# megvii-research/Far3D

Hardware: AMD Instinct MI355X
Metric: samples/sec (7-cam frame) end-to-end @ VoV-99 640x960 (higher is better)
Workload: dtype bf16x3; 1 GPU; BASELINE configs[1]: 7 cameras 3x640x960, VoV-99, A=1544 queries (644 learned + 644 adaptive + 256 propagated), 2312 self-attn keys, 6 decoder layers, streaming memory on, ego motion on; proposals=topk, fused_rows=True, parallelism=single GPU, weights=seeded random (far3d_amd.weights.init_state_dict, seed 0)

## Files before the change

### far3d_amd/csrc/conv_ws.hip

```cpp
#include "conv_ws.hpp"
#include "far3d_hip.h"

#ifdef FAR3D_PROFILING
std::atomic<int> g_ws_ablate{0};
extern "C" int far3d_conv_ws_set_ablate(int mask) { g_ws_ablate.store(mask); return 0; }
#endif

int far3d_conv_ws_launch(const IgemmParams& P, int tile, hipStream_t st) {
  switch (tile) {
    case 400: return launch_conv3x3_ws<2, 4, 2, 2, 4, true, true>(P, st);
    case 401: return launch_conv3x3_ws<1, 8, 2, 1, 4, true, true>(P, st);
    case 402: return launch_conv3x3_ws<1, 8, 5, 1, 4, true, false>(P, st);
    case 403: return launch_conv3x3_ws<2, 4, 3, 1, 4, true, true>(P, st);
    case 404: return launch_conv3x3_ws<2, 2, 1, 2, 2, true, true>(P, st);
    case 405: return launch_conv3x3_ws<2, 4, 2, 1, 4, true, true>(P, st);
    case 406: return launch_conv3x3_ws<2, 4, 1, 2, 4, true, true>(P, st);
    case 407: return launch_conv3x3_ws<1, 4, 5, 1, 2, true, false>(P, st);
    case 408: return launch_conv3x3_ws<1, 4, 3, 1, 2, true, true>(P, st);
    case 409: return launch_conv3x3_ws<2, 4, 2, 2, 2, true, true>(P, st);
    case 410: return launch_conv3x3_ws<2, 4, 2, 2, 4, true, true, 4>(P, st);
    case 411: return launch_conv3x3_ws<2, 4, 2, 1, 4, true, true, 6>(P, st);
    case 412: return launch_conv3x3_ws<2, 4, 1, 2, 4, true, true, 8>(P, st);
    case 413: return launch_conv3x3_ws<1, 8, 2, 1, 4, true, true, 8>(P, st);
    case 414: return launch_conv3x3_ws<1, 4, 5, 1, 2, true, false, 5>(P, st);
    case 415: return launch_conv3x3_ws<2, 2, 1, 2, 2, true, true, 6>(P, st);
    case 416: return launch_conv3x3_ws<2, 4, 3, 1, 4, true, true, 4>(P, st);
    case 417: return launch_conv3x3_ws<2, 4, 2, 1, 4, true, true, 4>(P, st);
    case 418: return launch_conv3x3_ws<4, 2, 2, 2, 4, true, true, 3>(P, st);
    case 419: return launch_conv3x3_ws<4, 2, 2, 1, 4, true, true, 3>(P, st);
    case 440: return launch_conv3x3_ws<2, 4, 2, 2, 4, true, true, 3, true>(P, st);
    case 444: return launch_conv3x3_ws<2, 2, 1, 2, 2, true, true, 3, true>(P, st);
    case 445: return launch_conv3x3_ws<2, 4, 2, 1, 4, true, true, 6, true>(P, st);
    case 450: return launch_conv3x3_ws<2, 4, 2, 1, 4, true, true, 6, false, 3>(P, st);
    case 451: return launch_conv3x3_ws<2, 4, 1, 2, 4, true, true, 6, false, 3>(P, st);
    case 452: return launch_conv3x3_ws<2, 4, 1, 2, 4, true, true, 9, false, 3>(P, st);
    case 453: return launch_conv3x3_ws<1, 8, 2, 1, 4, true, true, 6, false, 3>(P, st);
    case 454: return launch_conv3x3_ws<1, 8, 2, 1, 4, true, true, 9, false, 3>(P, st);
    case 455: return launch_conv3x3_ws<1, 7, 2, 1, 4, true, true, 9, false, 3>(P, st);
    case 456: return launch_conv3x3_ws<2, 7, 1, 1, 2, true, true, 9, false, 3>(P, st);
    case 457: return launch_conv3x3_ws<2, 2, 1, 2, 2, true, true, 6, false, 3>(P, st);
    case 458: return launch_conv3x3_ws<1, 4, 3, 1, 2, true, true, 6, false, 3>(P, st);
    case 459: return launch_conv3x3_ws<2, 4, 1, 1, 4, true, true, 9, false, 3>(P, st);
    case 420: return launch_conv3x3_ws<2, 4, 2, 2, 4, false, true>(P, st);
    case 421: return launch_conv3x3_ws<1, 8, 2, 1, 4, false, true>(P, st);
    case 422: return launch_conv3x3_ws<1, 8, 5, 1, 4, false, true>(P, st);
    case 423: return launch_conv3x3_ws<2, 4, 3, 1, 4, false, true>(P, st);
    default: break;
  }
  far3d_set_error("far3d_conv2d_nhwc: unknown wave-specialised tile %d", tile);
  return FAR3D_ERR_ARG;
}

int far3d_gemm_ws_launch(const IgemmParams& P, int tile, hipStream_t st) {
  switch (tile) {
    case 460: return launch_gemm1x1_ws<4, 2, 1, 2, 4, 4, 1>(P, st);
    case 461: return launch_gemm1x1_ws<4, 2, 1, 2, 4, 4, 2>(P, st);
    case 462: return launch_gemm1x1_ws<2, 4, 2, 1, 4, 4, 2>(P, st);
    case 463: return launch_gemm1x1_ws<2, 2, 2, 2, 4, 4, 2>(P, st);
    case 464: return launch_gemm1x1_ws<4, 2, 2, 2, 4, 3, 1>(P, st);
    case 465: return launch_gemm1x1_ws<4, 2, 1, 2, 2, 4, 2>(P, st);
    case 466: return launch_gemm1x1_ws<2, 2, 1, 2, 4, 6, 3>(P, st);
    case 467: return launch_gemm1x1_ws<2, 4, 1, 1, 4, 6, 2>(P, st);
    case 468: return launch_gemm1x1_ws<2, 2, 1, 2, 2, 3, 1>(P, st);
    case 469: return launch_gemm1x1_ws<4, 2, 1, 2, 4, 2, 1>(P, st);
    case 470: return launch_gemm1x1_ws<2, 4, 2, 2, 4, 3, 1>(P, st);
    case 471: return launch_gemm1x1_ws<2, 2, 4, 2, 4, 3, 1>(P, st);
    case 473: return launch_gemm1x1_ws<4, 2, 2, 2, 2, 3, 1>(P, st);
    case 474: return launch_gemm1x1_ws<3, 2, 2, 2, 4, 3, 1>(P, st);
    case 475: return launch_gemm1x1_ws<2, 2, 2, 2, 4, 4, 1>(P, st);
    case 476: return launch_gemm1x1_ws<2, 4, 2, 2, 2, 3, 1>(P, st);
    default: break;
  }
  far3d_set_error("far3d_conv2d_nhwc: unknown wave-specialised GEMM tile %d", tile);
  return FAR3D_ERR_ARG;
}

static int far3d_conv_ws_grouped_launch(const IgemmParams& P, const WsGroup& G, int tile, hipStream_t st) {
  switch (tile) {
    case 500: return launch_conv3x3_ws_grouped<2, 4, 2, 2, 4, true, true>(P, G, st);
    case 505: return launch_conv3x3_ws_grouped<2, 4, 2, 1, 4, true, true>(P, G, st);
    case 552: return launch_conv3x3_ws_grouped<2, 4, 1, 2, 4, true, true, 9, false, 3>(P, G, st);
    case 556: return launch_conv3x3_ws_grouped<2, 7, 1, 1, 2, true, true, 9, false, 3>(P, G, st);
    case 559: return launch_conv3x3_ws_grouped<2, 4, 1, 1, 4, true, true, 9, false, 3>(P, G, st);
    default: break;
  }
  far3d_set_error("far3d_conv2d_nhwc_grouped: unknown grouped tile %d", tile);
  return FAR3D_ERR_ARG;
}

extern "C" int far3d_conv2d_nhwc_grouped(const far3d_conv_problem* probs, int n, int tile, void* stream) {
  FAR3D_CHECK_ARG(probs && n >= 1 && n <= FAR3D_WS_GROUP_MAX, "far3d_conv2d_nhwc_grouped: %d problems (1..%d)", n, FAR3D_WS_GROUP_MAX);
  FAR3D_CHECK_ARG(tile >= 500 && tile < 560, "far3d_conv2d_nhwc_grouped: tile %d is not a grouped tile (500-559)", tile);
  auto aligned = [](const void* p, long a) { return ((uintptr_t)p % a) == 0; };
  WsGroup G;
  memset(&G, 0, sizeof(G));
  G.n = n;
  const int Cin = probs[0].Cin;
  for (int i = 0; i < n; ++i) {
    const far3d_conv_problem& c = probs[i];
    FAR3D_CHECK_ARG(c.Cin == Cin, "far3d_conv2d_nhwc_grouped: problem %d has Cin %d, problem 0 has %d (one Cin per launch)", i, c.Cin, Cin);
    FAR3D_CHECK_ARG(c.x && c.w && c.y && c.N > 0 && c.H > 0 && c.W > 0 && c.Cout > 0 && Cin > 0 && Cin % 32 == 0 && c.Cout % 32 == 0 &&
                    c.act >= 0 && c.act <= 2 && c.ldx >= 2 * Cin && c.ldy >= 2 * c.Cout &&
                    aligned(c.x, 16) && aligned(c.y, 16) && c.ldx % 8 == 0 && c.ldy % 8 == 0 && c.x_img_stride % 8 == 0 && c.y_img_stride % 8 == 0 &&
                    (long)c.N * c.H * c.W < (1L << 31) - 4096 && (long)c.H * c.W * c.ldx * 2 < 0x7fffffffL,
                    "far3d_conv2d_nhwc_grouped: problem %d: needs pair-stored maps in and out, Cin and Cout multiples of 32, 16-byte aligned rows "
                    "(N=%d H=%d W=%d Cin=%d Cout=%d ldx=%d ldy=%d act=%d)", i, c.N, c.H, c.W, c.Cin, c.Cout, c.ldx, c.ldy, c.act);
    FAR3D_CHECK_ARG(!c.y2 || (c.y2_scale && c.y2_shift && aligned(c.y2, 16) && aligned(c.y2_scale, 16) && aligned(c.y2_shift, 16) &&
                              c.ldy2 >= c.Cout && c.ldy2 % 4 == 0 && c.y2_img_stride % 4 == 0),
                    "far3d_conv2d_nhwc_grouped: problem %d: the second output is fp32 with 16-byte aligned rows, scale and shift", i);
    WsProblem& q = G.p[i];
    q.x = c.x; q.w = c.w; q.bias = c.bias; q.y = c.y;
    q.y2 = c.y2; q.y2_scale = c.y2_scale; q.y2_shift = c.y2_shift;
    q.x_img_stride = c.x_img_stride; q.y_img_stride = c.y_img_stride; q.y2_img_stride = c.y2_img_stride;
    q.N = c.N; q.H = c.H; q.W = c.W; q.ldx = c.ldx; q.ldy = c.ldy; q.ldy2 = c.ldy2; q.Cout = c.Cout; q.act = c.act;
  }
  IgemmParams P;
  memset(&P, 0, sizeof(P));
  const far3d_conv_problem& c0 = probs[0];
  P.x = c0.x; P.w = c0.w; P.bias = c0.bias; P.y = c0.y;
  P.x_img_stride = c0.x_img_stride; P.y_img_stride = c0.y_img_stride;
  P.N = c0.N; P.H = c0.H; P.W = c0.W; P.Cin = Cin; P.ldx = c0.ldx; P.Ho = c0.H; P.Wo = c0.W; P.Cout = c0.Cout; P.ldy = c0.ldy;
  P.KH = 3; P.KW = 3; P.stride = 1; P.pad = 1;
  P.cin_pad = Cin; P.nsteps = 9 * Cin / 32;
  P.act = c0.act; P.y_dt = FAR3D_DT_BF16_PAIR;
  const int rc = far3d_conv_ws_grouped_launch(P, G, tile, (hipStream_t)stream);
  if (rc != FAR3D_OK) return rc;
  FAR3D_CHECK_LAUNCH("far3d_conv2d_nhwc_grouped");
  return FAR3D_OK;
}
```

### far3d_amd/csrc/conv_ws.hpp

```cpp
#pragma once
#include "igemm_kernels.hpp"
#include <type_traits>

__device__ __forceinline__ __amdgpu_buffer_rsrc_t uniform_rsrc(const void* p, long nbytes) {
  const unsigned long long a = (unsigned long long)(uintptr_t)p;
  const unsigned lo = __builtin_amdgcn_readfirstlane((unsigned)a), hi = __builtin_amdgcn_readfirstlane((unsigned)(a >> 32));
  const int nb = __builtin_amdgcn_readfirstlane((int)(nbytes < 0x7fffffffL ? nbytes : 0x7fffffffL));
  return __builtin_amdgcn_make_buffer_rsrc((void*)(uintptr_t)(((unsigned long long)hi << 32) | lo), 0, nb, 0x00020000);
}

__device__ __forceinline__ void wait_vmcnt_dyn(int n) {
#define FAR3D_WVC(k) case k: wait_vmcnt<k>(); break;
  switch (n) {
    FAR3D_WVC(0) FAR3D_WVC(1) FAR3D_WVC(2) FAR3D_WVC(3) FAR3D_WVC(4) FAR3D_WVC(5) FAR3D_WVC(6) FAR3D_WVC(7) FAR3D_WVC(8)
    FAR3D_WVC(9) FAR3D_WVC(10) FAR3D_WVC(11) FAR3D_WVC(12) FAR3D_WVC(13) FAR3D_WVC(14) FAR3D_WVC(15) FAR3D_WVC(16)
    FAR3D_WVC(17) FAR3D_WVC(18) FAR3D_WVC(19) FAR3D_WVC(20) FAR3D_WVC(21) FAR3D_WVC(22) FAR3D_WVC(23) FAR3D_WVC(24)
    FAR3D_WVC(25) FAR3D_WVC(26) FAR3D_WVC(27) FAR3D_WVC(28) FAR3D_WVC(29) FAR3D_WVC(30) FAR3D_WVC(31) FAR3D_WVC(32)
    FAR3D_WVC(33) FAR3D_WVC(34) FAR3D_WVC(35) FAR3D_WVC(36) FAR3D_WVC(37) FAR3D_WVC(38) FAR3D_WVC(39) FAR3D_WVC(40)
    FAR3D_WVC(41) FAR3D_WVC(42) FAR3D_WVC(43) FAR3D_WVC(44) FAR3D_WVC(45) FAR3D_WVC(46) FAR3D_WVC(47)
    default: wait_vmcnt<48>(); break;
  }
#undef FAR3D_WVC
}

#ifdef FAR3D_PROFILING
extern std::atomic<int> g_ws_ablate;
#define FAR3D_WS_ABLATE_ARG g_ws_ablate.load(std::memory_order_relaxed)
#else
#define FAR3D_WS_ABLATE_ARG 0
#endif

struct WsProblem {
  const void* x; const void* w; const float* bias; void* y;
  float* y2; const float* y2_scale; const float* y2_shift;
  long x_img_stride, y_img_stride, y2_img_stride;
  int N, H, W, ldx, ldy, ldy2, Cout, act;
  int tiles_x, tiles_y, n_mt, item0;
};
struct WsGroup { WsProblem p[FAR3D_WS_GROUP_MAX]; int n; };
struct WsSingle {};

template <int WGM, int WGN, int WM, int WN, int NP, bool PAIR, bool DBUF, int NSW = 3, bool FLAGS = false, int GRP = 1, class GT = WsSingle>
__global__ __launch_bounds__(64 * (WGM * WGN + NP)) void conv3x3_ws_kernel(IgemmParams P, int tiles_x, int tiles_y, int n_mt, int n_items, int ablate,
                                                                          GT GP) {
#if defined(__HIP_DEVICE_COMPILE__)
  constexpr bool GROUPED = std::is_same<GT, WsGroup>::value;
  static_assert(!GROUPED || (PAIR && !FLAGS), "grouped launches: pair storage, barrier hand-over");
  constexpr int NWC = WGM * WGN;
  static_assert(NSW >= 3, "ring depth");
  static_assert(GRP == 1 || (GRP == 3 && (NSW == 6 || NSW == 9) && !FLAGS), "one barrier per tap, or per kernel row with a ring of 2 or 3 rows");
  constexpr int NG = NSW / GRP;
  constexpr int PLD = PAIR ? 2 : 1;
  constexpr int BM = 32 * WGM * WM, TH = WGN * WN, PW = 34, PH = TH + 2, PPIX = PW * PH;
  constexpr int PG = (PPIX + 15) / 16, PATCH_B = PG * 1024;
  constexpr int GA = BM / 16, WST = BM * 64, WSTAGE = PLD * WST;
  constexpr int PBASE = NSW * WSTAGE, PBUF = PLD * PATCH_B;
  constexpr int RB = WN + 2;
  constexpr int FLAGB = PBASE + 2 * PBUF;
  static_assert(FLAGB + (FLAGS ? 128 : 0) <= 163840, "LDS budget");
  static_assert(!FLAGS || (NP <= 4 && NWC <= 8), "flag words: one b128 read per 4 counters");
  extern __shared__ __attribute__((aligned(1024))) unsigned char smem[];
  [[maybe_unused]] volatile unsigned* const flg = reinterpret_cast<volatile unsigned*>(smem + FLAGB);
  if constexpr (FLAGS) {
    if (threadIdx.x < 32) flg[threadIdx.x] = 0u;
    __syncthreads();
  }
  [[maybe_unused]] bool gave_up = false;
  constexpr int SPIN_LIMIT = 1 << 18;
  const int t = threadIdx.x, lane = t & 63, wv = __builtin_amdgcn_readfirstlane(t >> 6);
  const int nchunks = P.cin_pad / 32;
  const int spt = 9 * nchunks;
  const int my_items = (n_items - (int)blockIdx.x + (int)gridDim.x - 1) / (int)gridDim.x;
  const int total_steps = my_items * spt, total_chunks = my_items * nchunks;
  const int Ktot = 9 * P.cin_pad * PLD;
  auto locate = [&](int item, int& q, int& li, int& txs, int& tys, int& nmt) __attribute__((always_inline)) {
    q = 0; li = item; txs = tiles_x; tys = tiles_y; nmt = n_mt;
    if constexpr (GROUPED) {
      for (int i = 1; i < GP.n; ++i) q += item >= GP.p[i].item0 ? 1 : 0;
      q = __builtin_amdgcn_readfirstlane(q);
      li = item - GP.p[q].item0; txs = GP.p[q].tiles_x; tys = GP.p[q].tiles_y; nmt = GP.p[q].n_mt;
    }
  };
#ifdef FAR3D_PROFILING
  if (P.prof && t == 0) {
    unsigned hw_, xcc_;
    asm volatile("s_getreg_b32 %0, hwreg(HW_REG_HW_ID)" : "=s"(hw_));
    asm volatile("s_getreg_b32 %0, hwreg(HW_REG_XCC_ID)" : "=s"(xcc_));
    P.prof[(long)blockIdx.x * 16 + 0] = (unsigned long long)hw_ | ((unsigned long long)xcc_ << 32);
    P.prof[(long)blockIdx.x * 16 + 6] = (unsigned long long)__builtin_amdgcn_s_memrealtime();
    P.prof[(long)blockIdx.x * 16 + 1] = (unsigned long long)__builtin_amdgcn_s_memtime();
    P.prof[(long)blockIdx.x * 16 + 4] = (unsigned long long)my_items;
  }
#endif

  if (wv >= NWC) {
    const int pw = wv - NWC;
    constexpr int GPL = (PG + NP - 1) / NP, GWL = (GA + NP - 1) / NP;
    const int rg = lane >> 2, pc = lane & 3;
    const int lc = pc ^ ((rg >> 2) & 3);
    int npq = (PG - pw + NP - 1) / NP, nwq = (GA - pw + NP - 1) / NP;
    npq = npq < 0 ? 0 : npq; nwq = nwq < 0 ? 0 : nwq;
    const int np = npq * PLD, nw = nwq * PLD;
    constexpr unsigned OOB = 0x80000000u;
    unsigned wvoff[GWL];
#pragma unroll
    for (int i = 0; i < GWL; ++i) wvoff[i] = (unsigned)((((pw + NP * i) * 16 + rg) * Ktot + lc * 8) * 2);
    long img_bytes = (long)P.H * P.W * P.ldx * 2;
    unsigned pvoff[GPL];
    const bf16_t* x_base = nullptr;
    const bf16_t* w_base = nullptr;
    long w_bytes = 0;
    auto decode = [&](int k, int& n, int& y0, int& x0, int& m0, int& q) __attribute__((always_inline)) {
      const int item = (int)blockIdx.x + k * (int)gridDim.x;
      int li, txs, tys, nmt;
      locate(item, q, li, txs, tys, nmt);
      const int mt = li % nmt, pt = li / nmt;
      const int tx = pt % txs, r = pt / txs;
      const int ty = r % tys;
      n = __builtin_amdgcn_readfirstlane(r / tys); y0 = __builtin_amdgcn_readfirstlane(ty * TH);
      x0 = __builtin_amdgcn_readfirstlane(tx * 32); m0 = __builtin_amdgcn_readfirstlane(mt * BM);
    };
    auto set_w_tile = [&](int k) __attribute__((always_inline)) {
      int n, y0, x0, m0, q;
      decode(k, n, y0, x0, m0, q);
      const void* w = P.w;
      int Cout = P.Cout;
      if constexpr (GROUPED) { w = GP.p[q].w; Cout = GP.p[q].Cout; }
      w_base = reinterpret_cast<const bf16_t*>(w) + (long)m0 * Ktot;
      w_bytes = w_tile_bytes(BM, m0, Cout, Ktot);
    };
    auto set_p_tile = [&](int k) __attribute__((always_inline)) {
      int n, y0, x0, m0, q;
      decode(k, n, y0, x0, m0, q);
      const void* x = P.x;
      long xis = P.x_img_stride;
      int H = P.H, W = P.W, ldx = P.ldx;
      if constexpr (GROUPED) {
        x = GP.p[q].x; xis = GP.p[q].x_img_stride; H = GP.p[q].H; W = GP.p[q].W; ldx = GP.p[q].ldx;
        img_bytes = (long)H * W * ldx * 2;
      }
      x_base = reinterpret_cast<const bf16_t*>(x) + (long)n * xis;
#pragma unroll
      for (int i = 0; i < GPL; ++i) {
        const int idx = (pw + NP * i) * 16 + rg;
        const int py = idx / PW, px = idx - py * PW;
        const int iy = y0 - 1 + py, ix = x0 - 1 + px;
        const bool ok = idx < PPIX && iy >= 0 && iy < H && ix >= 0 && ix < W;
        pvoff[i] = ok ? (unsigned)((((long)iy * W + ix) * ldx + lc * 8) * 2) : OOB;
      }
    };
    auto issue_w = [&](int step_in_tile, int stage) __attribute__((always_inline)) {
      const int c = step_in_tile / 9, tap = step_in_tile - 9 * c;
      const int kb = __builtin_amdgcn_readfirstlane((tap * P.cin_pad + c * 32) * PLD * 2);
      const __amdgpu_buffer_rsrc_t rs_w = uniform_rsrc(w_base, w_bytes);
      const int sbase = __builtin_amdgcn_readfirstlane(stage * WSTAGE);
#pragma unroll
      for (int i = 0; i < GWL; ++i) {
        if (i < nwq) {
#pragma unroll
          for (int pl = 0; pl < PLD; ++pl)
            __builtin_amdgcn_raw_ptr_buffer_load_lds(rs_w, (lds_void_t*)(smem + sbase + pl * WST + (pw + NP * i) * 1024), 16, wvoff[i],
                                                     kb + pl * 64, 0, 0);
        }
      }
    };
    auto issue_p = [&](int chunk_in_tile, int buf) __attribute__((always_inline)) {
      const __amdgpu_buffer_rsrc_t rs_x = uniform_rsrc(x_base, img_bytes);
      const int pbase = __builtin_amdgcn_readfirstlane(PBASE + buf * PBUF), coff = __builtin_amdgcn_readfirstlane(chunk_in_tile * (64 * PLD));
#pragma unroll
      for (int i = 0; i < GPL; ++i) {
        if (i < npq) {
#pragma unroll
          for (int pl = 0; pl < PLD; ++pl)
            __builtin_amdgcn_raw_ptr_buffer_load_lds(rs_x, (lds_void_t*)(smem + pbase + pl * PATCH_B + (pw + NP * i) * 1024), 16, pvoff[i],
                                                     coff + pl * 64, 0, 0);
        }
      }
    };
    int sw_step = 0, sw_tile = 0, sw_stage = 0;
    int gp_chunk = 0, gp_tile = 0, gp_buf = 0;
    int w_left = total_steps, p_left = total_chunks;
    set_w_tile(0); set_p_tile(0);
    auto next_w = [&]() __attribute__((always_inline)) {
      if (!(ablate & 1)) issue_w(sw_step, sw_stage);
      --w_left;
      sw_stage = sw_stage == NSW - 1 ? 0 : sw_stage + 1;
      if (++sw_step == spt) { sw_step = 0; ++sw_tile; if (w_left > 0) set_w_tile(sw_tile); }
    };
    auto next_p = [&]() __attribute__((always_inline)) {
      if (!(ablate & 1)) issue_p(gp_chunk, gp_buf);
      --p_left;
      gp_buf ^= 1;
      if (++gp_chunk == nchunks) { gp_chunk = 0; ++gp_tile; if (p_left > 0) set_p_tile(gp_tile); }
    };
    next_p();
#pragma unroll
    for (int i = 0; i < (NG - 1) * GRP; ++i)
      if (w_left > 0) next_w();
    const int total_groups = total_steps / GRP, gpc = 9 / GRP;
    int gic = 0;
    unsigned phist = 0;
    for (int g = 0; g < total_groups; ++g) {
      int ahead = total_groups - 1 - g;
      ahead = ahead > NG - 2 ? NG - 2 : ahead;
      const int cnt = ahead * GRP * nw + __builtin_popcount(phist & ((1u << (NG - 1)) - 1u)) * np;
      const int S = g * GRP;
      if (ablate & 1) wait_vmcnt<0>(); else wait_vmcnt_dyn(cnt);
      if constexpr (FLAGS) {
        if (lane == 0) flg[pw] = (unsigned)(S + 1);
        if (S > 0 && !(ablate & 8)) {
          for (int spins = 0; !gave_up; ++spins) {
            const u32x4_t c0 = *reinterpret_cast<volatile u32x4_t*>(smem + FLAGB + 64);
            u32x4_t c1 = c0;
            if constexpr (NWC > 4) c1 = *reinterpret_cast<volatile u32x4_t*>(smem + FLAGB + 80);
            unsigned m = c0.x;
            if constexpr (NWC > 1) m = min(m, c0.y);
            if constexpr (NWC > 2) m = min(m, c0.z);
            if constexpr (NWC > 3) m = min(m, c0.w);
            if constexpr (NWC > 4) m = min(m, c1.x);
            if constexpr (NWC > 5) m = min(m, c1.y);
            if constexpr (NWC > 6) m = min(m, c1.z);
            if constexpr (NWC > 7) m = min(m, c1.w);
            if (__builtin_amdgcn_readfirstlane(m) >= (unsigned)S) break;
            if (spins > SPIN_LIMIT) gave_up = true;
            __builtin_amdgcn_s_sleep(2);
          }
        }
      } else {
#ifdef FAR3D_PROFILING
        if (!(ablate & 8))
#endif
        __builtin_amdgcn_s_barrier();
      }
      asm volatile("" ::: "memory");
#pragma unroll
      for (int i = 0; i < GRP; ++i)
        if (w_left > 0) next_w();
      phist <<= 1;
      if (gic == 0 && p_left > 0) { next_p(); phist |= 1u; }
      gic = gic == gpc - 1 ? 0 : gic + 1;
    }
    return;
  }

  const int wm = wv / WGN, wn = wv % WGN, l31 = lane & 31, hi = lane >> 5;
  int aaddr[WM], baddr[RB][3];
#pragma unroll
  for (int i = 0; i < WM; ++i) {
    const int r = (wm * WM + i) * 32 + l31;
    aaddr[i] = r * 64 + ((hi ^ ((r >> 2) & 3)) << 4);
  }
#pragma unroll
  for (int r = 0; r < RB; ++r)
#pragma unroll
    for (int kx = 0; kx < 3; ++kx) {
      const int idx = (wn * WN + r) * PW + l31 + kx;
      baddr[r][kx] = PBASE + idx * 64 + ((hi ^ ((idx >> 2) & 3)) << 4);
    }
  f32x16_t acc[WM][WN];
  u32x4_t fa[2][PLD][WM], fb[2][PLD][WN];

  auto load_a = [&](int set, int soff, int kk) __attribute__((always_inline)) {
#ifdef FAR3D_PROFILING
    if (ablate & 4) return;
#endif
    const int x32 = kk * 32;
#pragma unroll
    for (int pl = 0; pl < PLD; ++pl)
#pragma unroll
      for (int i = 0; i < WM; ++i) fa[set][pl][i] = *reinterpret_cast<const u32x4_t*>(smem + pl * WST + ((aaddr[i] ^ x32) + soff));
  };
  auto load_b = [&](int set, int tap, int kk) __attribute__((always_inline)) {
#ifdef FAR3D_PROFILING
    if (ablate & 4) return;
#endif
    const int ky = tap / 3, kx = tap - 3 * ky, x32 = kk * 32;
#pragma unroll
    for (int pl = 0; pl < PLD; ++pl)
#pragma unroll
      for (int j = 0; j < WN; ++j) fb[set][pl][j] = *reinterpret_cast<const u32x4_t*>(smem + pl * PATCH_B + (baddr[j + ky][kx] ^ x32));
  };
  auto load_set = [&](int set, int soff, int tap, int kk) __attribute__((always_inline)) { load_a(set, soff, kk); load_b(set, tap, kk); };
  auto mma_term = [&](int set, int term) __attribute__((always_inline)) {
    const int pa = (PAIR && term == 0) ? 1 : 0, pb = (PAIR && term == 1) ? 1 : 0;
#pragma unroll
    for (int i = 0; i < WM; ++i)
#pragma unroll
      for (int j = 0; j < WN; ++j) mma<bf16_t>(acc[i][j], fa[set][pa][i], fb[set][pb][j]);
  };
  auto mma_set = [&](int set) __attribute__((always_inline)) {
    if constexpr (PAIR) { mma_term(set, 0); mma_term(set, 1); }
    mma_term(set, 2);
  };

  int G = 0;
  int soff = 0;
  [[maybe_unused]] int Sg = 0;
  [[maybe_unused]] u32x4_t pfl = {0u, 0u, 0u, 0u};
#ifdef FAR3D_PROFILING
  unsigned long long pf_ta = 0, pf_tb = 0, pf_wait = 0, pf_body = 0, pf_epi = 0;
  const bool pf_on = P.prof != nullptr && wv == 0;
#endif
  for (int k = 0; k < my_items; ++k) {
    const int item = (int)blockIdx.x + k * (int)gridDim.x;
    int prob, li, txs, tys, nmt;
    locate(item, prob, li, txs, tys, nmt);
    const int mt = li % nmt, pt = li / nmt;
    const int tx = pt % txs, rr = pt / txs;
    const int ty = rr % tys, n = rr / tys;
    const int x0 = tx * 32, y0 = ty * TH, m0 = mt * BM;
#pragma unroll
    for (int i = 0; i < WM; ++i)
#pragma unroll
      for (int j = 0; j < WN; ++j)
#pragma unroll
        for (int r = 0; r < 16; ++r) acc[i][j][r] = 0.f;

    for (int c = 0; c < nchunks; ++c, ++G) {
#pragma unroll
      for (int tap = 0; tap < 9; ++tap) {
        const int stage = soff;
        if (tap % GRP == 0) {
        __builtin_amdgcn_s_waitcnt(0xc07f);
#ifdef FAR3D_PROFILING
        if (pf_on) {
          const unsigned long long now = __builtin_amdgcn_s_memtime();
          if (pf_tb) { pf_wait += pf_tb - pf_ta; pf_body += now - pf_tb; }
          pf_ta = now;
        }
#endif
        if constexpr (FLAGS) {
          if (lane == 0) flg[16 + wv] = (unsigned)Sg;
          if (!(ablate & 8)) {
            for (int spins = 0; !gave_up; ++spins) {
              unsigned m = pfl.x;
              if constexpr (NP > 1) m = min(m, pfl.y);
              if constexpr (NP > 2) m = min(m, pfl.z);
              if constexpr (NP > 3) m = min(m, pfl.w);
              if (__builtin_amdgcn_readfirstlane(m) >= (unsigned)(Sg + 1)) break;
              if (spins > SPIN_LIMIT) gave_up = true;
              __builtin_amdgcn_s_sleep(1);
              pfl = *reinterpret_cast<volatile u32x4_t*>(smem + FLAGB);
            }
          }
          ++Sg;
        } else {
#ifdef FAR3D_PROFILING
          if (!(ablate & 8))
#endif
          __builtin_amdgcn_s_barrier();
        }
        asm volatile("" ::: "memory");
        __builtin_amdgcn_sched_barrier(0);
#ifdef FAR3D_PROFILING
        if (pf_on) pf_tb = __builtin_amdgcn_s_memtime();
        if (tap == 0 && c == 0 && k == 0 && P.prof && t == 0) P.prof[(long)blockIdx.x * 16 + 2] = (unsigned long long)__builtin_amdgcn_s_memtime();
#endif
        }
        if (ablate & 2) { soff = soff == (NSW - 1) * WSTAGE ? 0 : soff + WSTAGE; continue; }
        if constexpr (DBUF) {
          load_set(0, stage, tap, 0);
          __builtin_amdgcn_sched_barrier(0);
          if (tap > 0 || c > 0) mma_set(1);
          __builtin_amdgcn_sched_barrier(0);
          load_a(1, stage, 1);
          if constexpr (FLAGS) pfl = *reinterpret_cast<volatile u32x4_t*>(smem + FLAGB);
          __builtin_amdgcn_sched_barrier(0);
          if constexpr (PAIR) {
            mma_term(0, 0);
            __builtin_amdgcn_sched_barrier(0);
            load_b(1, tap, 1);
            __builtin_amdgcn_sched_barrier(0);
            mma_term(0, 1);
            mma_term(0, 2);
          } else {
            load_b(1, tap, 1);
            __builtin_amdgcn_sched_barrier(0);
            mma_term(0, 2);
          }
          __builtin_amdgcn_sched_barrier(0);
          soff = soff == (NSW - 1) * WSTAGE ? 0 : soff + WSTAGE;
        } else {
          load_set(0, stage, tap, 0);
          __builtin_amdgcn_sched_barrier(0);
          mma_set(0);
          __builtin_amdgcn_sched_barrier(0);
          load_set(0, stage, tap, 1);
          if constexpr (FLAGS) pfl = *reinterpret_cast<volatile u32x4_t*>(smem + FLAGB);
          __builtin_amdgcn_sched_barrier(0);
          mma_set(0);
          __builtin_amdgcn_sched_barrier(0);
          soff = soff == (NSW - 1) * WSTAGE ? 0 : soff + WSTAGE;
        }
      }
      const int d = (G & 1) ? -PBUF : PBUF;
#pragma unroll
      for (int r = 0; r < RB; ++r)
#pragma unroll
        for (int kx = 0; kx < 3; ++kx) baddr[r][kx] += d;
    }
    if constexpr (DBUF) mma_set(1);
    __builtin_amdgcn_sched_barrier(0);
#ifdef FAR3D_PROFILING
    unsigned long long pf_e0 = 0;
    if (pf_on) {
      pf_e0 = __builtin_amdgcn_s_memtime();
      if (pf_tb) { pf_wait += pf_tb - pf_ta; pf_body += pf_e0 - pf_tb; pf_tb = 0; }
    }
#endif

    {
      const int px = x0 + l31;
      void* y = P.y;
      const float* bias = P.bias;
      long yis = P.y_img_stride;
      int Ho = P.Ho, Wo = P.Wo, ldy = P.ldy, Cout = P.Cout, act = P.act;
      [[maybe_unused]] float* y2 = nullptr;
      [[maybe_unused]] const float *y2s = nullptr, *y2h = nullptr;
      [[maybe_unused]] long y2is = 0;
      [[maybe_unused]] int ldy2 = 0;
      if constexpr (GROUPED) {
        const WsProblem& pq = GP.p[prob];
        y = pq.y; bias = pq.bias; yis = pq.y_img_stride; Ho = pq.H; Wo = pq.W; ldy = pq.ldy; Cout = pq.Cout; act = pq.act;
        y2 = pq.y2; y2s = pq.y2_scale; y2h = pq.y2_shift; y2is = pq.y2_img_stride; ldy2 = pq.ldy2;
      }
      unsigned char* yb = reinterpret_cast<unsigned char*>(y);
#pragma unroll
      for (int j = 0; j < WN; ++j) {
        const int py = y0 + wn * WN + j;
        const bool ok = py < Ho && px < Wo;
        const long pix_b = ((long)n * yis + ((long)py * Wo + px) * ldy) * 2;
#pragma unroll
        for (int i = 0; i < WM; ++i) {
          const int cb = m0 + (wm * WM + i) * 32;
          if (cb >= Cout) continue;
#pragma unroll
          for (int qp = 0; qp < 2; ++qp) {
            uint2 h[2], l[2];
#pragma unroll
            for (int u = 0; u < 2; ++u) {
              const int q = 2 * qp + u;
              float4 b4 = make_float4(0.f, 0.f, 0.f, 0.f);
              if (bias) b4 = *reinterpret_cast<const float4*>(bias + cb + 8 * q + 4 * hi);
              float v[4];
#pragma unroll
              for (int e = 0; e < 4; ++e) v[e] = acc[i][j][4 * q + e];
              v[0] += b4.x; v[1] += b4.y; v[2] += b4.z; v[3] += b4.w;
              if (act == ACT_RELU) {
#pragma unroll
                for (int e = 0; e < 4; ++e) v[e] = fmaxf(v[e], 0.f);
              } else if (act == ACT_SWISH) {
                if constexpr (PAIR) {
#pragma unroll
                  for (int e = 0; e < 4; ++e) v[e] = v[e] * (1.f / (1.f + expf(-v[e])));
                } else {
#pragma unroll
                  for (int e = 0; e < 4; ++e) v[e] = v[e] * __frcp_rn(1.f + __expf(-v[e]));
                }
              }
              if constexpr (GROUPED) {
                if (y2 && ok) {
                  const int m = cb + 8 * q + 4 * hi;
                  const long so = (long)n * Cout + m;
                  float w4[4];
#pragma unroll
                  for (int e = 0; e < 4; ++e) w4[e] = y2s[so + e] * v[e] + y2h[so + e];
                  *reinterpret_cast<float4*>(y2 + n * y2is + ((long)py * Wo + px) * ldy2 + m) = make_float4(w4[0], w4[1], w4[2], w4[3]);
                }
              }
              if constexpr (PAIR) split4f(v[0], v[1], v[2], v[3], h[u], l[u]);
              else { h[u] = make_uint2(pack_bf16x2(v[0], v[1]), pack_bf16x2(v[2], v[3])); l[u] = make_uint2(0u, 0u); }
            }
            u32x4_t oh, ol;
            {
              const auto sx = __builtin_amdgcn_permlane32_swap(h[0].x, h[1].x, false, false);
              const auto sy = __builtin_amdgcn_permlane32_swap(h[0].y, h[1].y, false, false);
              oh = u32x4_t{sx[0], sy[0], sx[1], sy[1]};
            }
            const int qoff = (2 * qp + hi) * 16;
            if constexpr (PAIR) {
              const auto sx = __builtin_amdgcn_permlane32_swap(l[0].x, l[1].x, false, false);
              const auto sy = __builtin_amdgcn_permlane32_swap(l[0].y, l[1].y, false, false);
              ol = u32x4_t{sx[0], sy[0], sx[1], sy[1]};
              if (ok) {
                unsigned char* d = yb + pix_b + (long)(cb >> 5) * 128 + qoff;
                *reinterpret_cast<u32x4_t*>(d) = oh;
                *reinterpret_cast<u32x4_t*>(d + 64) = ol;
              }
            } else {
              if (ok) *reinterpret_cast<u32x4_t*>(yb + pix_b + (long)cb * 2 + qoff) = oh;
            }
          }
        }
      }
    }
#ifdef FAR3D_PROFILING
    if (pf_on) pf_epi += __builtin_amdgcn_s_memtime() - pf_e0;
#endif
  }
#ifdef FAR3D_PROFILING
  if (P.prof && t == 0) {
    P.prof[(long)blockIdx.x * 16 + 3] = (unsigned long long)__builtin_amdgcn_s_memtime();
    P.prof[(long)blockIdx.x * 16 + 7] = (unsigned long long)__builtin_amdgcn_s_memrealtime();
    P.prof[(long)blockIdx.x * 16 + 5] = (unsigned long long)total_steps;
    P.prof[(long)blockIdx.x * 16 + 8] = pf_wait; P.prof[(long)blockIdx.x * 16 + 9] = pf_body; P.prof[(long)blockIdx.x * 16 + 10] = pf_epi;
  }
#endif
#endif
}

template <int WGM, int WGN, int WM, int WN, int NP, int NSW, int GRP, bool SUMS>
__global__ __launch_bounds__(64 * (WGM * WGN + NP)) void gemm1x1_ws_kernel(IgemmParams P, int npt, int nct, int ablate) {
#if defined(__HIP_DEVICE_COMPILE__)
  constexpr int NWC = WGM * WGN;
  constexpr int BM = 32 * WGM * WM, BP = 32 * WGN * WN;
  constexpr int GA = BM / 16, GB = BP / 16, SLOTS = GA + GB;
  static_assert(SLOTS % NP == 0, "every producer issues the same number of pieces per step (counted vmcnt)");
  constexpr int SPW = SLOTS / NP;
  constexpr int SUB = (BM + BP) * 64, STAGE = 2 * SUB;
  static_assert(NSW % GRP == 0 && NSW / GRP >= 2, "ring = at least two hand-over groups");
  constexpr int NG = NSW / GRP;
  extern __shared__ __attribute__((aligned(1024))) unsigned char smem[];
  const int t = threadIdx.x, lane = t & 63, wv = __builtin_amdgcn_readfirstlane(t >> 6);
  constexpr int SUMB = NSW * STAGE;
  static_assert(SUMB + 4 * BM * 8 <= 163840, "LDS budget");
  [[maybe_unused]] long long* const lsum = reinterpret_cast<long long*>(smem + SUMB);
  constexpr bool do_sums = SUMS;
  if (do_sums) {
    for (int i = threadIdx.x; i < 4 * BM; i += 64 * (NWC + NP)) lsum[i] = 0;
    __syncthreads();
  }
  const int HoWo = P.Ho * P.Wo;
  const long Npix = (long)P.N * HoWo;
  const int nsteps = P.cin_pad / 32;
  const int Ktot = P.cin_pad * 2;
  const int xcd = (int)blockIdx.x & 7, slot0 = (int)blockIdx.x >> 3, dslot = (int)gridDim.x >> 3;
  const int vslots = ((npt - xcd + 7) >> 3) * nct;
  const int my_items = vslots > slot0 ? (vslots - slot0 + dslot - 1) / dslot : 0;
  const int total_steps = my_items * nsteps;
  const int total_groups = (total_steps + GRP - 1) / GRP;
  auto decode = [&](int k, int& p0, int& m0) __attribute__((always_inline)) {
    const int slot = slot0 + k * dslot;
    const int ct = slot % nct, pt = (slot / nct) * 8 + xcd;
    p0 = __builtin_amdgcn_readfirstlane(pt * BP); m0 = __builtin_amdgcn_readfirstlane(ct * BM);
  };

  if (wv >= NWC) {
    const int pw = wv - NWC;
    const int rg = lane >> 2, pc = lane & 3;
    const int lc = pc ^ ((rg >> 2) & 3);
    constexpr unsigned OOB = 0x80000000u;
    const long x_bytes = ((long)(P.N - 1) * P.x_img_stride + (long)HoWo * P.ldx) * 2;
    unsigned voff[SPW];
    int sdst[SPW];
    bool isw[SPW];
#pragma unroll
    for (int i = 0; i < SPW; ++i) {
      const int q = pw + NP * i;
      isw[i] = q < GA;
      const int g = isw[i] ? q : q - GA;
      sdst[i] = (isw[i] ? 0 : BM * 64) + g * 1024;
      voff[i] = isw[i] ? (unsigned)(((g * 16 + rg) * Ktot + lc * 8) * 2) : 0u;
    }
    const bf16_t* w_base = nullptr;
    long w_bytes = 0;
    int cur_tile = 0, cur_step = 0, cur_stage = 0, left = total_steps;
    auto set_tile = [&](int k) __attribute__((always_inline)) {
      int p0, m0;
      decode(k, p0, m0);
      w_base = reinterpret_cast<const bf16_t*>(P.w) + (long)m0 * Ktot;
      w_bytes = w_tile_bytes(BM, m0, P.Cout, Ktot);
#pragma unroll
      for (int i = 0; i < SPW; ++i) {
        if (!isw[i]) {
          const int g = pw + NP * i - GA;
          const long p = (long)p0 + g * 16 + rg;
          if (p < Npix) {
            int n, rem;
            pix_split(p, HoWo, n, rem);
            voff[i] = (unsigned)(((long)n * P.x_img_stride + (long)rem * P.ldx + lc * 8) * 2);
          } else {
            voff[i] = OOB;
          }
        }
      }
    };
    auto next = [&]() __attribute__((always_inline)) {
      if (!(ablate & 1)) {
        const __amdgpu_buffer_rsrc_t rs_w = uniform_rsrc(w_base, w_bytes);
        const __amdgpu_buffer_rsrc_t rs_x = uniform_rsrc(P.x, x_bytes);
        const int sbase = __builtin_amdgcn_readfirstlane(cur_stage * STAGE);
        const int kb = __builtin_amdgcn_readfirstlane(cur_step * 128);
#pragma unroll
        for (int i = 0; i < SPW; ++i) {
#pragma unroll
          for (int pl = 0; pl < 2; ++pl) {
            if (isw[i])
              __builtin_amdgcn_raw_ptr_buffer_load_lds(rs_w, (lds_void_t*)(smem + sbase + pl * SUB + sdst[i]), 16, voff[i], kb + pl * 64, 0, 0);
            else
              __builtin_amdgcn_raw_ptr_buffer_load_lds(rs_x, (lds_void_t*)(smem + sbase + pl * SUB + sdst[i]), 16, voff[i], kb + pl * 64, 0, 0);
          }
        }
      }
      --left;
      cur_stage = cur_stage == NSW - 1 ? 0 : cur_stage + 1;
      if (++cur_step == nsteps) { cur_step = 0; ++cur_tile; if (left > 0) set_tile(cur_tile); }
    };
    if (my_items > 0) set_tile(0);
#pragma unroll
    for (int i = 0; i < (NG - 1) * GRP; ++i)
      if (left > 0) next();
    for (int g = 0; g < total_groups; ++g) {
      int later = total_steps - (g + 1) * GRP;
      later = later < 0 ? 0 : (later > (NG - 2) * GRP ? (NG - 2) * GRP : later);
      if (ablate & 1) wait_vmcnt<0>(); else wait_vmcnt_dyn(later * SPW * 2);
      __builtin_amdgcn_s_barrier();
      asm volatile("" ::: "memory");
#pragma unroll
      for (int i = 0; i < GRP; ++i)
        if (left > 0) next();
    }
    if (do_sums) __builtin_amdgcn_s_barrier();
    return;
  }

  const int wm = wv / WGN, wn = wv % WGN, l31 = lane & 31, hi = lane >> 5;
  int aaddr[WM], baddr[WN];
#pragma unroll
  for (int i = 0; i < WM; ++i) {
    const int r = (wm * WM + i) * 32 + l31;
    aaddr[i] = r * 64 + ((hi ^ ((r >> 2) & 3)) << 4);
  }
#pragma unroll
  for (int j = 0; j < WN; ++j) {
    const int r = (wn * WN + j) * 32 + l31;
    baddr[j] = BM * 64 + r * 64 + ((hi ^ ((r >> 2) & 3)) << 4);
  }
  f32x16_t acc[WM][WN];
  u32x4_t fa[2][2][WM], fb[2][2][WN];
  auto load_a = [&](int set, int soff, int kk) __attribute__((always_inline)) {
    const int x32 = kk * 32;
#pragma unroll
    for (int pl = 0; pl < 2; ++pl)
#pragma unroll
      for (int i = 0; i < WM; ++i) fa[set][pl][i] = *reinterpret_cast<const u32x4_t*>(smem + pl * SUB + ((aaddr[i] ^ x32) + soff));
  };
  auto load_b = [&](int set, int soff, int kk) __attribute__((always_inline)) {
    const int x32 = kk * 32;
#pragma unroll
    for (int pl = 0; pl < 2; ++pl)
#pragma unroll
      for (int j = 0; j < WN; ++j) fb[set][pl][j] = *reinterpret_cast<const u32x4_t*>(smem + pl * SUB + ((baddr[j] ^ x32) + soff));
  };
  auto mma_term = [&](int set, int term) __attribute__((always_inline)) {
    const int pa = term == 0 ? 1 : 0, pb = term == 1 ? 1 : 0;
#pragma unroll
    for (int i = 0; i < WM; ++i)
#pragma unroll
      for (int j = 0; j < WN; ++j) mma<bf16_t>(acc[i][j], fa[set][pa][i], fb[set][pb][j]);
  };
  int soff = 0, gs = 0;
  [[maybe_unused]] int flush_tile = 0, gcount = 0;
  auto flush = [&](int T) __attribute__((always_inline)) {
    int fp0, fm0;
    decode(T, fp0, fm0);
    const int fcam0 = (int)((long)fp0 / P.sums_hw);
    long long* src = lsum + (T & 1) * 2 * BM;
    for (int i = wv * 64 + lane; i < 2 * BM; i += 64 * NWC) {
      const int sl = i / BM, chn = i - sl * BM, cam = fcam0 + sl;
      const long long v = src[i];
      if (v != 0) {
        src[i] = 0;
        if (cam < P.N && fm0 + chn < P.Cout)
          atomicAdd(reinterpret_cast<unsigned long long*>(P.chan_sums + (long)cam * P.Cout + fm0 + chn), (unsigned long long)v);
      }
    }
  };
  for (int k = 0; k < my_items; ++k) {
    int p0, m0;
    decode(k, p0, m0);
#pragma unroll
    for (int i = 0; i < WM; ++i)
#pragma unroll
      for (int j = 0; j < WN; ++j)
#pragma unroll
        for (int r = 0; r < 16; ++r) acc[i][j][r] = 0.f;
    for (int s = 0; s < nsteps; ++s) {
      const int stage = soff;
      if (gs == 0) {
        __builtin_amdgcn_s_waitcnt(0xc07f);
        __builtin_amdgcn_s_barrier();
        asm volatile("" ::: "memory");
        __builtin_amdgcn_sched_barrier(0);
        if constexpr (do_sums) {
          while (flush_tile < k && ((flush_tile + 1) * nsteps - 1) / GRP < gcount) { flush(flush_tile); ++flush_tile; }
          ++gcount;
        }
      }
      gs = gs == GRP - 1 ? 0 : gs + 1;
      if (ablate & 2) { soff = soff == (NSW - 1) * STAGE ? 0 : soff + STAGE; continue; }
      load_a(0, stage, 0); load_b(0, stage, 0);
      __builtin_amdgcn_sched_barrier(0);
      if (s > 0) { mma_term(1, 0); mma_term(1, 1); mma_term(1, 2); }
      __builtin_amdgcn_sched_barrier(0);
      load_a(1, stage, 1);
      __builtin_amdgcn_sched_barrier(0);
      mma_term(0, 0);
      __builtin_amdgcn_sched_barrier(0);
      load_b(1, stage, 1);
      __builtin_amdgcn_sched_barrier(0);
      mma_term(0, 1);
      mma_term(0, 2);
      __builtin_amdgcn_sched_barrier(0);
      soff = soff == (NSW - 1) * STAGE ? 0 : soff + STAGE;
    }
    if (!(ablate & 2)) { mma_term(1, 0); mma_term(1, 1); mma_term(1, 2); }
    __builtin_amdgcn_sched_barrier(0);

    {
      unsigned char* yb = reinterpret_cast<unsigned char*>(P.y);
      const int cam0 = do_sums ? (int)((long)p0 / P.sums_hw) : 0;
      const long bnd = (long)(cam0 + 1) * P.sums_hw;
      const bool two = do_sums && (long)p0 + BP > bnd;
      long pix_b[WN];
      bool okj[WN], secj[WN];
#pragma unroll
      for (int j = 0; j < WN; ++j) {
        const long p = (long)p0 + (wn * WN + j) * 32 + l31;
        okj[j] = p < Npix;
        secj[j] = p >= bnd;
        pix_b[j] = 0;
        if (okj[j]) {
          int n, rem;
          pix_split(p, HoWo, n, rem);
          pix_b[j] = ((long)n * P.y_img_stride + (long)rem * P.ldy) * 2;
        }
      }
      auto stored = [&](int i, int j, int q, int cb, uint2& h, uint2& l) __attribute__((always_inline)) {
        float4 b4 = make_float4(0.f, 0.f, 0.f, 0.f);
        if (P.bias) b4 = *reinterpret_cast<const float4*>(P.bias + cb + 8 * q + 4 * hi);
        float v[4];
#pragma unroll
        for (int e = 0; e < 4; ++e) v[e] = acc[i][j][4 * q + e];
        v[0] += b4.x; v[1] += b4.y; v[2] += b4.z; v[3] += b4.w;
        if (P.act == ACT_RELU) {
#pragma unroll
          for (int e = 0; e < 4; ++e) v[e] = fmaxf(v[e], 0.f);
        } else if (P.act == ACT_SWISH) {
#pragma unroll
          for (int e = 0; e < 4; ++e) v[e] = v[e] * (1.f / (1.f + expf(-v[e])));
        }
        split4f(v[0], v[1], v[2], v[3], h, l);
      };
      auto quantise = [&](const uint2& h, const uint2& l, int q, int (&qs)[16], float& mx) __attribute__((always_inline)) {
        const unsigned w4[4] = {h.x, h.y, l.x, l.y};
#pragma unroll
        for (int e = 0; e < 2; ++e) {
          const float h0 = __uint_as_float(w4[e] << 16), h1 = __uint_as_float(w4[e] & 0xffff0000u);
          const float l0 = __uint_as_float(w4[2 + e] << 16), l1 = __uint_as_float(w4[2 + e] & 0xffff0000u);
          mx = fmaxf(mx, fmaxf(fabsf(h0), fabsf(h1)));
          qs[4 * q + 2 * e] += __float2int_rn(h0 * (float)(1 << FAR3D_SUMS_FRAC_BITS)) + __float2int_rn(l0 * (float)(1 << FAR3D_SUMS_FRAC_BITS));
          qs[4 * q + 2 * e + 1] += __float2int_rn(h1 * (float)(1 << FAR3D_SUMS_FRAC_BITS)) + __float2int_rn(l1 * (float)(1 << FAR3D_SUMS_FRAC_BITS));
        }
      };
      auto half_sum = [&](int x) __attribute__((always_inline)) -> int {
        x += __builtin_amdgcn_update_dpp(0, x, 0x128, 0xf, 0xf, true);
        x += __builtin_amdgcn_update_dpp(0, x, 0x124, 0xf, 0xf, true);
        x += __builtin_amdgcn_update_dpp(0, x, 0x122, 0xf, 0xf, true);
        x += __builtin_amdgcn_update_dpp(0, x, 0x121, 0xf, 0xf, true);
        typedef unsigned u2_t __attribute__((ext_vector_type(2)));
        const u2_t r = __builtin_amdgcn_permlane16_swap((unsigned)x, (unsigned)x, false, false);
        const unsigned rx = r.x, ry = r.y;
        return (int)(rx + ry);
      };
      auto reduce_add = [&](const int (&qs)[16], float mx, int sl, int cb) __attribute__((always_inline)) {
        const bool wide = WN > 2 || __any(mx >= (float)(1 << (24 - FAR3D_SUMS_FRAC_BITS)));
        long long* dst = lsum + ((k & 1) * 2 + sl) * BM + (cb - m0) + 4 * hi;
#pragma unroll
        for (int r = 0; r < 16; ++r) {
          long long tot;
          if (!wide) {
            tot = (long long)half_sum(qs[r]);
          } else {
            const int lo16 = qs[r] & 0xffff, hi16 = qs[r] >> 16;
            tot = (long long)half_sum(hi16) * 65536ll + (long long)half_sum(lo16);
          }
          if (l31 == 0 && tot != 0) atomicAdd(reinterpret_cast<unsigned long long*>(dst + 8 * (r >> 2) + (r & 3)), (unsigned long long)tot);
        }
      };
      auto channel_block = [&](auto ic) __attribute__((always_inline)) {
        constexpr int i = decltype(ic)::value;
        const int cb = m0 + (wm * WM + i) * 32;
        if (cb >= P.Cout) return;
        int qs[16];
        float mx = 0.f;
#pragma unroll
        for (int r = 0; r < 16; ++r) qs[r] = 0;
#pragma unroll
        for (int j = 0; j < WN; ++j) {
#pragma unroll
          for (int qp = 0; qp < 2; ++qp) {
            uint2 h[2], l[2];
#pragma unroll
            for (int u = 0; u < 2; ++u) {
              stored(i, j, 2 * qp + u, cb, h[u], l[u]);
              if (do_sums && okj[j] && !secj[j]) quantise(h[u], l[u], 2 * qp + u, qs, mx);
            }
            u32x4_t oh, ol;
            {
              const auto sx = __builtin_amdgcn_permlane32_swap(h[0].x, h[1].x, false, false);
              const auto sy = __builtin_amdgcn_permlane32_swap(h[0].y, h[1].y, false, false);
              oh = u32x4_t{sx[0], sy[0], sx[1], sy[1]};
            }
            {
              const auto sx = __builtin_amdgcn_permlane32_swap(l[0].x, l[1].x, false, false);
              const auto sy = __builtin_amdgcn_permlane32_swap(l[0].y, l[1].y, false, false);
              ol = u32x4_t{sx[0], sy[0], sx[1], sy[1]};
            }
            if (okj[j]) {
              unsigned char* d = yb + pix_b[j] + (long)(cb >> 5) * 128 + (2 * qp + hi) * 16;
              *reinterpret_cast<u32x4_t*>(d) = oh;
              *reinterpret_cast<u32x4_t*>(d + 64) = ol;
            }
          }
        }
        if constexpr (do_sums) {
          auto exact_add = [&](int sl) __attribute__((always_inline)) {
            long long* dst = lsum + ((k & 1) * 2 + sl) * BM + (cb - m0) + 4 * hi;
#pragma unroll
            for (int q = 0; q < 4; ++q) {
              long long x[4] = {0, 0, 0, 0};
#pragma unroll
              for (int j = 0; j < WN; ++j) {
                uint2 h, l;
                stored(i, j, q, cb, h, l);
                if (okj[j] && secj[j] == (sl == 1)) {
                  const unsigned w4[4] = {h.x, h.y, l.x, l.y};
#pragma unroll
                  for (int e = 0; e < 2; ++e) {
                    const float h0 = __uint_as_float(w4[e] << 16), h1 = __uint_as_float(w4[e] & 0xffff0000u);
                    const float l0 = __uint_as_float(w4[2 + e] << 16), l1 = __uint_as_float(w4[2 + e] & 0xffff0000u);
                    x[2 * e] += __double2ll_rn((double)h0 * (double)(1 << FAR3D_SUMS_FRAC_BITS)) + __double2ll_rn((double)l0 * (double)(1 << FAR3D_SUMS_FRAC_BITS));
                    x[2 * e + 1] += __double2ll_rn((double)h1 * (double)(1 << FAR3D_SUMS_FRAC_BITS)) + __double2ll_rn((double)l1 * (double)(1 << FAR3D_SUMS_FRAC_BITS));
                  }
                }
              }
#pragma unroll
              for (int e = 0; e < 4; ++e) {
                const long long v = x[e];
                const long long tot = (long long)half_sum((int)(v & 0xffff)) + ((long long)half_sum((int)((v >> 16) & 0xffff)) << 16) +
                                      ((long long)half_sum((int)((v >> 32) & 0xffff)) << 32) + ((long long)half_sum((int)(v >> 48)) << 48);
                if (l31 == 0 && tot != 0) atomicAdd(reinterpret_cast<unsigned long long*>(dst + 8 * q + e), (unsigned long long)tot);
              }
            }
          };
          const bool huge = __any(mx >= 2048.f);
          if (huge) exact_add(0); else reduce_add(qs, mx, 0, cb);
          if (two) {
            float mx1 = 0.f;
#pragma unroll
            for (int r = 0; r < 16; ++r) qs[r] = 0;
#pragma unroll
            for (int j = 0; j < WN; ++j)
#pragma unroll
              for (int q = 0; q < 4; ++q) {
                uint2 h, l;
                stored(i, j, q, cb, h, l);
                if (okj[j] && secj[j]) quantise(h, l, q, qs, mx1);
              }
            if (__any(mx1 >= 2048.f)) exact_add(1); else reduce_add(qs, mx1, 1, cb);
          }
        }
      };
      static_assert(WM <= 4, "channel blocks per consumer");
      channel_block(std::integral_constant<int, 0>{});
      if constexpr (WM > 1) channel_block(std::integral_constant<int, 1>{});
      if constexpr (WM > 2) channel_block(std::integral_constant<int, 2>{});
      if constexpr (WM > 3) channel_block(std::integral_constant<int, 3>{});
    }
  }
  if constexpr (do_sums) {
    __builtin_amdgcn_s_waitcnt(0xc07f);
    __builtin_amdgcn_s_barrier();
    asm volatile("" ::: "memory");
    while (flush_tile < my_items) { flush(flush_tile); ++flush_tile; }
  }
#endif
}

template <int WGM, int WGN, int WM, int WN, int NP, int NSW, int GRP>
static int launch_gemm1x1_ws(const IgemmParams& P, hipStream_t st) {
  constexpr int BM = 32 * WGM * WM, BP = 32 * WGN * WN;
  constexpr size_t lds = (size_t)NSW * 2 * (BM + BP) * 64 + 4 * BM * 8;
  static_assert(lds <= 163840, "LDS budget");
  const long Npix = (long)P.N * P.Ho * P.Wo;
  const int npt = (int)((Npix + BP - 1) / BP), nct = (P.Cout + BM - 1) / BM;
  static std::atomic<unsigned long long> lds_ok_s{0};
  static std::atomic<int> n_cu{0};
  int cus = n_cu.load(std::memory_order_relaxed);
  if (cus == 0) {
    int dev = 0;
    if (hipGetDevice(&dev) != hipSuccess) dev = 0;
    if (hipDeviceGetAttribute(&cus, hipDeviceAttributeMultiprocessorCount, dev) != hipSuccess || cus <= 0) cus = 256;
    n_cu.store(cus, std::memory_order_relaxed);
  }
  constexpr int wg_per_cu = lds <= 81920 && 64 * (WGM * WGN + NP) <= 1024 ? 2 : 1;
  const long items = (long)((npt + 7) / 8 * 8) * nct;
  long grid = (long)cus * wg_per_cu;
  grid = (grid + 7) / 8 * 8;
  if (items < grid) grid = items;
  static std::atomic<unsigned long long> lds_ok{0};
  if constexpr (lds > 65536)
    if (const int rc = far3d_allow_lds(P.chan_sums ? reinterpret_cast<const void*>(&gemm1x1_ws_kernel<WGM, WGN, WM, WN, NP, NSW, GRP, true>)
                                                   : reinterpret_cast<const void*>(&gemm1x1_ws_kernel<WGM, WGN, WM, WN, NP, NSW, GRP, false>),
                                       (int)lds, P.chan_sums ? lds_ok_s : lds_ok, "far3d_conv2d_nhwc")) return rc;
  if (P.chan_sums) {
    if (P.sums_hw < BP || P.cin_pad / 32 < 2 * GRP) {
      far3d_set_error("far3d_conv2d_nhwc: channel sums on this wave-specialised GEMM tile need Ho*Wo (%d) >= %d pixels and Cin >= %d", P.sums_hw, BP, 64 * GRP);
      return FAR3D_ERR_ARG;
    }
    hipLaunchKernelGGL((gemm1x1_ws_kernel<WGM, WGN, WM, WN, NP, NSW, GRP, true>), dim3((unsigned)grid), dim3(64 * (WGM * WGN + NP)), lds, st, P, npt, nct, FAR3D_WS_ABLATE_ARG);
  } else {
    hipLaunchKernelGGL((gemm1x1_ws_kernel<WGM, WGN, WM, WN, NP, NSW, GRP, false>), dim3((unsigned)grid), dim3(64 * (WGM * WGN + NP)), lds, st, P, npt, nct, FAR3D_WS_ABLATE_ARG);
  }
  return 0;
}

template <int WGM, int WGN, int WM, int WN, int NP, bool PAIR, bool DBUF, int NSW = 3, bool FLAGS = false, int GRP = 1>
static int launch_conv3x3_ws(const IgemmParams& P, hipStream_t st) {
  constexpr int BM = 32 * WGM * WM, TH = WGN * WN, PLD = PAIR ? 2 : 1;
  constexpr int PG = (34 * (TH + 2) + 15) / 16;
  constexpr size_t lds = (size_t)NSW * PLD * BM * 64 + (size_t)2 * PLD * PG * 1024 + (FLAGS ? 128 : 0);
  static_assert(lds <= 163840, "LDS budget");
  const int tiles_x = (P.Wo + 31) / 32, tiles_y = (P.Ho + TH - 1) / TH, n_mt = (P.Cout + BM - 1) / BM;
  const int n_items = P.N * tiles_x * tiles_y * n_mt;
  static std::atomic<int> n_cu{0};
  int cus = n_cu.load(std::memory_order_relaxed);
  if (cus == 0) {
    int dev = 0;
    if (hipGetDevice(&dev) != hipSuccess) dev = 0;
    if (hipDeviceGetAttribute(&cus, hipDeviceAttributeMultiprocessorCount, dev) != hipSuccess || cus <= 0) cus = 256;
    n_cu.store(cus, std::memory_order_relaxed);
  }
  constexpr int wg_per_cu = lds <= 81920 && 64 * (WGM * WGN + NP) <= 1024 ? 2 : 1;
  const int grid = n_items < cus * wg_per_cu ? n_items : cus * wg_per_cu;
  static std::atomic<unsigned long long> lds_ok{0};
  if constexpr (lds > 65536)
    if (const int rc = far3d_allow_lds(reinterpret_cast<const void*>(&conv3x3_ws_kernel<WGM, WGN, WM, WN, NP, PAIR, DBUF, NSW, FLAGS, GRP>), (int)lds, lds_ok, "far3d_conv2d_nhwc")) return rc;
  hipLaunchKernelGGL((conv3x3_ws_kernel<WGM, WGN, WM, WN, NP, PAIR, DBUF, NSW, FLAGS, GRP>), dim3((unsigned)grid), dim3(64 * (WGM * WGN + NP)), lds, st, P, tiles_x, tiles_y, n_mt,
                     n_items, FAR3D_WS_ABLATE_ARG, WsSingle{});
  return 0;
}

template <int WGM, int WGN, int WM, int WN, int NP, bool PAIR, bool DBUF, int NSW = 3, bool FLAGS = false, int GRP = 1>
static int launch_conv3x3_ws_grouped(const IgemmParams& P, const WsGroup& G0, hipStream_t st) {
  constexpr int BM = 32 * WGM * WM, TH = WGN * WN, PLD = PAIR ? 2 : 1;
  constexpr int PG = (34 * (TH + 2) + 15) / 16;
  constexpr size_t lds = (size_t)NSW * PLD * BM * 64 + (size_t)2 * PLD * PG * 1024 + (FLAGS ? 128 : 0);
  static_assert(lds <= 163840, "LDS budget");
  WsGroup G = G0;
  long items[FAR3D_WS_GROUP_MAX];
  for (int i = 0; i < G.n; ++i) {
    WsProblem& q = G.p[i];
    q.tiles_x = (q.W + 31) / 32; q.tiles_y = (q.H + TH - 1) / TH; q.n_mt = (q.Cout + BM - 1) / BM;
    items[i] = (long)q.N * q.tiles_x * q.tiles_y * q.n_mt;
  }
  for (int i = 1; i < G.n; ++i)
    for (int j = i; j > 0 && items[j] > items[j - 1]; --j) {
      const WsProblem t = G.p[j]; G.p[j] = G.p[j - 1]; G.p[j - 1] = t;
      const long u = items[j]; items[j] = items[j - 1]; items[j - 1] = u;
    }
  long n_items = 0;
  for (int i = 0; i < G.n; ++i) { G.p[i].item0 = (int)n_items; n_items += items[i]; }
  if (n_items >= (1L << 31) - 4096) { far3d_set_error("far3d_conv2d_nhwc_grouped: %ld items", n_items); return FAR3D_ERR_ARG; }
  static std::atomic<int> n_cu{0};
  int cus = n_cu.load(std::memory_order_relaxed);
  if (cus == 0) {
    int dev = 0;
    if (hipGetDevice(&dev) != hipSuccess) dev = 0;
    if (hipDeviceGetAttribute(&cus, hipDeviceAttributeMultiprocessorCount, dev) != hipSuccess || cus <= 0) cus = 256;
    n_cu.store(cus, std::memory_order_relaxed);
  }
  constexpr int wg_per_cu = lds <= 81920 && 64 * (WGM * WGN + NP) <= 1024 ? 2 : 1;
  const int grid = n_items < cus * wg_per_cu ? (int)n_items : cus * wg_per_cu;
  static std::atomic<unsigned long long> lds_ok{0};
  if constexpr (lds > 65536)
    if (const int rc = far3d_allow_lds(reinterpret_cast<const void*>(&conv3x3_ws_kernel<WGM, WGN, WM, WN, NP, PAIR, DBUF, NSW, FLAGS, GRP, WsGroup>), (int)lds, lds_ok,
                                       "far3d_conv2d_nhwc_grouped")) return rc;
  hipLaunchKernelGGL((conv3x3_ws_kernel<WGM, WGN, WM, WN, NP, PAIR, DBUF, NSW, FLAGS, GRP, WsGroup>), dim3((unsigned)grid), dim3(64 * (WGM * WGN + NP)), lds, st, P,
                     G.p[0].tiles_x, G.p[0].tiles_y, G.p[0].n_mt, (int)n_items, FAR3D_WS_ABLATE_ARG, G);
  return 0;
}
```

### far3d_amd/lib.py

```python
import ctypes
import os

os.environ.setdefault("GPU_MAX_HW_QUEUES", "8")

import torch

_HERE = os.path.dirname(os.path.abspath(__file__))
LIB_PATH = os.path.join(_HERE, "libfar3d_hip.so")

c_int, c_float, c_void_p, c_char_p = ctypes.c_int, ctypes.c_float, ctypes.c_void_p, ctypes.c_char_p
c_long = ctypes.c_long
_p = c_void_p

SIGNATURES = {
    "far3d_last_error": (c_char_p, []),
    "far3d_abi_version": (c_int, []),
    "far3d_device_count": (c_int, []),
    "far3d_device_arch": (c_int, [c_int, c_char_p, c_int]),
    "far3d_msda_forward": (c_int, [_p, c_int, _p, _p, _p, _p, _p] + [c_int] * 7 + [_p]),
    "far3d_aggregate_forward": (c_int, [_p, c_int, _p, _p, _p, _p, _p, _p, _p, _p, c_int] + [c_int] * 7 +
                                [_p, _p, _p, c_float, c_float, c_int, c_int, c_int, _p, _p, c_int, _p, _p]),
    "far3d_conv2d_nhwc": (c_int, [_p, c_int, _p, c_int, _p, _p, c_int] + [c_int] * 5 + [c_long] + [c_int] * 4 +
                          [c_long] + [c_int] * 5 + [_p, c_int, c_int, c_long, c_int, c_int] +
                          [_p, c_int, c_int, c_long, _p, _p, _p, c_int, _p]),
    "far3d_conv2d_nhwc_grouped": (c_int, [_p, c_int, c_int, _p]),
    "far3d_attention_forward": (c_int, [_p, _p, _p, c_int, _p, c_int] + [c_int] * 8 + [c_float, _p, c_int, c_int, _p]),
    "far3d_attention_f32_variant": (c_int, [c_int]),
    "far3d_layernorm": (c_int, [_p, _p, _p, _p, c_int, c_int, c_int, c_int, c_float, c_int, _p, c_int, _p, c_int, c_int, _p, c_int, c_int, _p]),
    "far3d_layernorm_rows": (c_int, [_p, _p, _p, _p, c_int, c_int, c_int, c_int, c_float, c_int, _p, c_int, _p, c_int, c_int, _p, c_int, c_int, _p, _p]),
    "far3d_rowchain_attn_out": (c_int, [_p, c_int, _p, c_int, _p, c_int, _p, _p, _p, _p, _p, _p, c_int, _p, c_int, _p, c_int,
                                        _p, c_int, c_float, _p]),
    "far3d_rowchain_ffn": (c_int, [_p, c_int, _p, c_int, _p, c_int] + [_p] * 12 + [_p, c_int, _p, c_int, _p, c_int, c_int, c_float, _p]),
    "far3d_rowchain_qkv": (c_int, [_p, c_int, _p, c_int, _p, _p, _p, c_int, c_int, _p]),
    "far3d_rowchain_branches": (c_int, [_p, c_int] + [_p] * 10 + [c_int] + [_p] * 6 + [c_int, _p, c_int, _p, c_int, c_int, c_float, _p]),
    "far3d_ese_nhwc": (c_int, [_p, c_int, _p, _p, _p, _p, _p, c_int, c_int, c_int, c_int, c_long, c_int, c_long,
                               c_int, c_long, _p, _p]),
    "far3d_ese_fused_nhwc": (c_int, [_p, c_int, _p, _p, _p, _p, _p, _p, c_int, c_int, c_int, c_int, c_int, c_long, c_int, c_long, c_int, c_long,
                                     c_int, c_int, c_int, c_long, _p, _p]),
    "far3d_cam_embed_chain": (c_int, [_p] * 10 + [c_int, c_int, c_int, c_int, c_float, c_int, _p]),
    "far3d_groupnorm_nhwc": (c_int, [_p, c_int, _p, _p, _p, _p, c_int, c_int, c_int, c_int, c_float, c_int, _p]),
    "far3d_maxpool3x3s2_nhwc": (c_int, [_p, c_int, _p] + [c_int] * 7 + [c_long, _p]),
    "far3d_stem_im2col": (c_int, [_p, _p, c_int, c_int, c_int, c_int, _p]),
    "far3d_stem_conv": (c_int, [_p, _p, _p, _p, c_int, c_int, c_int, c_int, c_long, c_int, _p]),
    "far3d_proposal_select": (c_int, [_p, _p, c_int, c_int, c_int, c_int, _p, _p, _p, _p, _p, _p, c_int, c_float, c_int, _p]),
    "far3d_proposal_gather": (c_int, [_p, c_int, c_int, c_int, _p, _p, _p, _p, c_int, _p, _p, c_int, c_int, c_int, c_int,
                                      c_float, c_float, c_int, _p, _p, c_int, c_int, _p, c_float, _p, _p, _p, _p, c_int, _p, _p, _p]),
    "far3d_proposal_gather_md": (c_int, [_p, c_int, c_int, c_int, _p, _p, _p, _p, c_int, _p, _p, c_int, c_int, c_int, c_int,
                                         c_float, c_float, c_int, _p, _p, c_int, c_int, _p, c_float, _p, _p, _p, _p, c_int,
                                         c_int, c_int, _p, _p, _p]),
    "far3d_proposal_extra_rows": (c_int, [_p, c_int, c_int, c_int, c_int, _p, _p, _p, c_float, c_float, c_int, _p, c_int,
                                          _p, _p, _p, _p, c_int, c_int, _p, _p, _p]),
    "far3d_compact_rows": (c_int, [_p, _p, c_int, c_int, c_int, _p, c_int, _p, _p, _p]),
    "far3d_row_affine_ln": (c_int, [_p, _p, _p, _p, _p] + [c_int] * 6 + [c_float, c_int, _p]),
    "far3d_posemb3d": (c_int, [_p, _p, _p, c_int, _p]),
    "far3d_memory_prepare": (c_int, [_p] * 9 + [c_float, c_int, _p, c_int, c_int, c_int] + [_p] * 9),
    "far3d_head_finalize": (c_int, [_p] * 5 + [c_int] * 4 + [_p, _p, c_int, c_int, _p]),
    "far3d_memory_post_update": (c_int, [_p] * 10 + [c_int] * 4 + [_p] * 6),
    "far3d_add_cast": (c_int, [_p, _p, _p, c_int, _p, c_int, c_int, c_int, c_long, c_long, _p]),
    "far3d_agg_order": (c_int, [_p, _p, _p, c_int, c_int, _p, c_float, c_float, _p, c_int, c_int, c_int, _p, _p, c_int, c_int, c_int, _p, _p, _p]),
    "far3d_agg_tables": (c_int, [_p, _p, c_int, c_int, c_int, _p]),
    "far3d_topk": (c_int, [_p, c_int, c_int, _p, _p, _p]),
    "far3d_decode_topk": (c_int, [_p, _p, c_int, c_int, c_int, c_int, _p, _p, _p, _p, _p, _p, c_long, _p]),
    "far3d_decode_topk_mem": (c_int, [_p, _p, c_int, c_int, c_int, c_int, _p, _p, _p, _p, _p, _p, c_long, _p, c_int, c_int, _p, _p]),
    "far3d_camera_prep": (c_int, [_p, _p, _p, _p, _p, c_int, _p]),
    "far3d_nan_to_num": (c_int, [_p, _p, c_long, _p]),
    "far3d_image_resample_h": (c_int, [_p, c_long, c_int, c_int, _p, _p, _p, c_int, c_int, c_int, c_int, c_int, _p]),
    "far3d_image_resample_v": (c_int, [_p, c_int, c_int, c_int, _p, _p, c_int, c_int, c_int, c_int, c_int, _p, c_int, c_int, c_int,
                                       _p, _p, c_int, _p]),
}

_lib = None


class Far3dHipError(RuntimeError):
    pass


def load():
    global _lib
    if _lib is not None:
        return _lib
    if not os.path.exists(LIB_PATH):
        raise Far3dHipError(
            "libfar3d_hip.so not found at %s -- run `python -c 'import __graft_entry__ as g; g.build()'` "
            "(or `python far3d_amd/build.py`). There is no CPU fallback for the Far3D hot path." % LIB_PATH)
    lib = ctypes.CDLL(LIB_PATH)
    for name, (res, args) in SIGNATURES.items():
        fn = getattr(lib, name)
        fn.restype = res
        fn.argtypes = args
    _lib = lib
    return lib


def check(status, what):
    if status != 0:
        msg = load().far3d_last_error()
        raise Far3dHipError("%s failed (code %d): %s" % (what, status, msg.decode() if msg else "?"))


def require_device():
    lib = load()
    if lib.far3d_device_count() <= 0:
        raise Far3dHipError("far3d_amd needs a HIP device (MI355X / gfx950); none is visible and there is "
                            "no CPU fallback. The CPU restatement lives in oracle/ and is test-only.")
    return lib
```

### include/far3d_hip.h

```cpp
#ifndef FAR3D_HIP_H
#define FAR3D_HIP_H
#include <stdint.h>

#ifdef __cplusplus
extern "C" {
#endif

#define FAR3D_DT_F32 0
#define FAR3D_DT_BF16 1
#define FAR3D_DT_F32_BF16X3 2
#define FAR3D_DT_BF16_PAIR 3
#define FAR3D_SUMS_MAX_PARTS 32
#define FAR3D_SUMS_FRAC_BITS 18
#define FAR3D_SUMS_SCRATCH_FLOATS(N, C) ((long)(N) * (C) * (2 * FAR3D_SUMS_MAX_PARTS + 1))

#define FAR3D_OK 0
#define FAR3D_ERR_ARG (-1)
#define FAR3D_ERR_LAUNCH (-2)
#define FAR3D_ERR_UNSUPPORTED (-3)

const char* far3d_last_error(void);
int far3d_abi_version(void);
int far3d_device_count(void);
int far3d_device_arch(int dev, char* buf, int buflen);

int far3d_msda_forward(const void* value, int value_dtype, const int64_t* spatial_shapes,
                       const int64_t* level_start_index, const float* sampling_loc,
                       const float* attn_weight, float* out, int bs, int S, int H, int Dh, int L, int Q,
                       int P, void* stream);

int far3d_aggregate_forward(const void* feat, int feat_dtype, const float* ref, const float* offsets,
                            const float* lidar2img, const float* U, const float* Vc, const float* cam_tables,
                            const int32_t* perm, void* out, int out_dt, int A,
                            int N, int S, int C, int G, int P, int L, const int32_t* level_hw,
                            const int32_t* level_start, const float* pc_range, float pad_h, float pad_w,
                            int ldU, int ldOffs, int variant, float* split_partials, int32_t* split_tickets, int split_extra,
                            const float* qbase, void* stream);
#define FAR3D_AGG_LISTS_FLOATS(A) ((long)(((A) + 7) / 8 * 8) * (2L * 1024 * 9 + 8))

int far3d_agg_tables(const float* Vc, float* tables, int layers, int N, int J, void* stream);

int far3d_conv2d_nhwc(const void* x, int x_dt, const void* w, int w_dt, const float* bias, void* y, int y_dt,
                      int N, int H, int W, int Cin, int ldx, long x_img_stride, int Ho, int Wo, int Cout, int ldy,
                      long y_img_stride, int KH, int KW, int stride, int pad, int act, const void* res, int res_dt,
                      int ldr, long res_img_stride, int Hr, int Wr, void* y2, int y2_dt, int ldy2,
                      long y2_img_stride, const float* y2_scale, const float* y2_shift, long long* chan_sums, int tile,
                      void* stream);

typedef struct {
  const void* x;
  const void* w;
  const float* bias;
  void* y;
  float* y2;
  const float* y2_scale;
  const float* y2_shift;
  long x_img_stride, y_img_stride, y2_img_stride;
  int N, H, W, Cin, Cout, ldx, ldy, ldy2;
  int act;
} far3d_conv_problem;
#define FAR3D_WS_GROUP_MAX 16

int far3d_conv2d_nhwc_grouped(const far3d_conv_problem* probs, int n, int tile, void* stream);

int far3d_attention_forward(const void* q, const void* k, const void* v, int dtype, void* out, int out_dt, int Aq, int Nk,
                            int heads, int head_dim, int ldq, int ldk, int ldv, int ldo, float scale,
                            const int32_t* hole_count, int hole_start, int hole_end, void* stream);

int far3d_attention_f32_variant(int variant);

int far3d_layernorm(const float* x, const float* gamma, const float* beta, float* y, int rows, int C, int ldx,
                    int ldy, float eps, int act, const float* add, int lda, void* y2, int ldy2, int y2_dt, void* yb, int ldyb,
                    int yb_dt, void* stream);
int far3d_layernorm_rows(const float* x, const float* gamma, const float* beta, float* y, int rows, int C, int ldx,
                         int ldy, float eps, int act, const float* add, int lda, void* y2, int ldy2, int y2_dt, void* yb, int ldyb,
                         int yb_dt, const int32_t* out_rows, void* stream);

int far3d_rowchain_attn_out(const void* att, int ld_att, const float* x, int ldx, const float* qpos, int ldq,
                            const void* w_out, const float* b_out, const float* g0, const float* be0,
                            const void* w_wl, const float* b_wl, int n_wl, float* x1, int ldx1, float* ul, int ldu,
                            const int32_t* ul_rows, int M, float eps, void* stream);

int far3d_rowchain_ffn(const void* agg, int ld_agg, const float* x1, int ldx1, const float* qpos, int ldq,
                       const void* w_o, const float* b_o, const float* g1, const float* be1,
                       const void* w_1, const float* b_1, const void* w_2, const float* b_2,
                       const float* g2, const float* be2, const void* w_qkv, const float* b_qkv,
                       float* out, int ldo, void* qkv, int ldqkv, void* xop, int ldxop, int M, float eps, void* stream);

int far3d_rowchain_qkv(const float* x, int ldx, const float* qpos, int ldq, const void* w_qkv, const float* b_qkv,
                       void* qkv, int ldqkv, int M, void* stream);

int far3d_rowchain_branches(const void* h, int ldh, const void* w_c0, const float* b_c0, const float* g_c0, const float* be_c0,
                            const void* w_c1, const float* b_c1, const float* g_c1, const float* be_c1,
                            const void* w_c2, const float* b_c2, int n_cls, const void* w_r0, const float* b_r0,
                            const void* w_r1, const float* b_r1, const void* w_r2, const float* b_r2, int n_reg,
                            float* cls, int ld_cls, float* reg, int ld_reg, int M, float eps, void* stream);

int far3d_ese_nhwc(const void* x, int dt, const float* fcw, const float* fcb, const void* identity, void* y,
                   float* scratch, int N, int HW, int C, int ldx, long x_img_stride, int ldi, long i_img_stride,
                   int ldy, long y_img_stride, long long* chan_sums, void* stream);

int far3d_ese_fused_nhwc(const void* x, int dt, const float* fcw, const float* fcb, const void* identity, void* y, void* pooled,
                         float* gate, int N, int H, int W, int C, int ldx, long x_img_stride, int ldi,
                         long i_img_stride, int ldy, long y_img_stride, int Hp, int Wp, int ldp, long p_img_stride,
                         long long* chan_sums, void* stream);

int far3d_groupnorm_nhwc(const void* x, int dt, const float* gamma, const float* beta, void* y, float* scratch, int N,
                         int HW, int C, int groups, float eps, int relu, void* stream);

int far3d_maxpool3x3s2_nhwc(const void* x, int dt, void* y, int N, int H, int W, int C, int Ho, int Wo, int ldy,
                            long y_img_stride, void* stream);

int far3d_stem_im2col(const float* img, void* out, int out_dt, int N, int H, int W, void* stream);

int far3d_stem_conv(const float* img, const void* w, const float* bias, void* y, int N, int H, int W, int ldy, long y_img_stride,
                    int act, void* stream);

int far3d_proposal_select(const float* const* cls, const float* const* reg, int ncls, int nreg, int N, int L,
                          const int32_t* level_hw, const int32_t* strides, float* scratch_sw, float* weights, int* sel_idx,
                          int* sel_cnt, int cap, float thr, int mode, void* stream);

int far3d_proposal_gather(const float* const* reg, int nreg, int N, int L, const int32_t* level_hw, const int32_t* strides,
                          const int* sel_idx, const int* sel_cnt, int cap, const float* weights,
                          const float* depth_logit, int hd, int wd, int nd, int depth_stride, float depth_min,
                          float depth_max, int depth_bins, const float* img2lidar, const void* feat, int feat_dt, int C,
                          const float* pc_range, float score_thr, float* ref2d, float* ctx, float* box2d, float* score,
                          int rows_total, int32_t* m_out, int32_t* overflow_out, void* stream);

int far3d_proposal_gather_md(const float* const* reg, int nreg, int N, int L, const int32_t* level_hw, const int32_t* strides,
                             const int* sel_idx, const int* sel_cnt, int cap, const float* weights,
                             const float* depth_logit, int hd, int wd, int nd, int depth_stride, float depth_min,
                             float depth_max, int depth_bins, const float* img2lidar, const void* feat, int feat_dt, int C,
                             const float* pc_range, float score_thr, float* ref2d, float* ctx, float* box2d, float* score,
                             int primary_rows, int topk, int range_min_bin, int32_t* md_flags, int32_t* md_info, void* stream);

int far3d_proposal_extra_rows(const int* sel_cnt, int N, int sel_cap, int primary_rows, int topk, const int32_t* md_flags,
                              const int32_t* md_info, const float* img2lidar, float depth_min, float depth_max, int depth_bins,
                              const float* pc_range, int C, float* ref2d, float* ctx, float* box2d, float* score, int rows_total,
                              int fill_hole, int32_t* m_out, int32_t* overflow_out, void* stream);

int far3d_compact_rows(const float* src, const int32_t* counts, int nblocks, int rows_per_block, int D, float* dst, int dst_rows,
                       int32_t* m_out, int32_t* overflow_out, void* stream);

int far3d_row_affine_ln(const float* x, const float* gamma, const float* beta, const float* add, float* y, int rows, int C,
                        int ldx, int ldg, int lda, int ldy, float eps, int do_ln, void* stream);


int far3d_posemb3d(const float* pos, const float* dim_t128, float* out, int R, void* stream);

int far3d_memory_prepare(const float* emb, const float* ref, const double* ts, const float* pose, const float* velo,
                         const float* ego_pose_inv, const double* timestamp, const float* pseudo_ref, const float* dim_t256,
                         float prev_exists, int fresh, const float* pc_range, int L, int E, int P, float* m_emb, float* m_ref,
                         double* m_ts, float* m_pose, float* m_velo, float* temp_ref, float* nerf, float* tpos, void* stream);

int far3d_head_finalize(const float* reg, const float* ref, float* cls_all, float* box, float* score, int layers, int A,
                        int code_size, int num_classes, const float* pc_range, const int32_t* hole_count, int hole_start, int hole_end,
                        void* stream);

int far3d_memory_post_update(const float* m_emb, const float* m_ref, const double* m_ts, const float* m_pose, const float* m_velo,
                             const int64_t* topk_idx, const float* dec_last, const float* box_last, const float* ego_pose,
                             const double* timestamp, int L, int E, int K, int code_size, float* emb, float* ref, double* ts,
                             float* pose, float* velo, void* stream);

int far3d_add_cast(const float* a, const float* b, void* out_sum, int sum_dt, void* out_a, int a_dt, int rows, int C, long ld_sum,
                   long ld_a, void* stream);

int far3d_agg_order(const float* ref, const float* lidar2img, int32_t* perm, int A, int N, const float* pc_range, float pad_h,
                    float pad_w, const int32_t* hole_count, int hole_start, int hole_end, int row_base,
                    const float* Vc, float* tables, int layers, int J, int split_extra, int32_t* inv, float* qbase, void* stream);

int far3d_topk(const float* vals, int n, int K, int64_t* idx_out, float* val_out, void* stream);

#define FAR3D_DECODE_WS_BYTES(n, K) ((((long)(n) + 40959) / 40960) * (long)(K) * 8)
int far3d_decode_topk(const float* cls_last, const float* box_last, int A, int num_classes, int code_size, int K,
                      const float* post_center_range, float* boxes, float* scores, int64_t* labels, unsigned char* keep,
                      void* workspace, long workspace_bytes, void* stream);
int far3d_decode_topk_mem(const float* cls_last, const float* box_last, int A, int num_classes, int code_size, int K,
                          const float* post_center_range, float* boxes, float* scores, int64_t* labels, unsigned char* keep,
                          void* workspace, long workspace_bytes, const float* mem_scores, int mem_n, int mem_K,
                          int64_t* mem_idx_out, void* stream);

int far3d_camera_prep(const float* lidar2img, const float* intrinsics, const float* extrinsics, float* img2lidar, float* c14,
                      int N, void* stream);

int far3d_nan_to_num(float* x, void* bf16_copy, long n, void* stream);

int far3d_cam_embed_chain(const float* l2i, const float* w0t, const float* b0, const float* w2t, const float* b2,
                          const float* ln_g, const float* ln_b, const float* w3t, const float* b3, float* out, int N, int L,
                          int J, int Hd, float eps, int ld_l2i, void* stream);

int far3d_image_resample_h(const unsigned char* src, long src_pitch, int in_h, int in_w, unsigned char* dst, const int32_t* bounds,
                           const int32_t* coeffs, int ksize, int row0, int rows, int x0, int outw, void* stream);
int far3d_image_resample_v(const unsigned char* tmp, int row0, int rows, int outw, const int32_t* bounds, const int32_t* coeffs,
                           int ksize, int y0, int outh, int flip, int mode, void* out, int out_dt, int pad_h, int pad_w,
                           const float* mean, const float* stdinv, int to_rgb, void* stream);

#ifdef __cplusplus
}
#endif
#endif
```

Before: 72.26 samples/s.

## Defer conv epilogue across items and deal partial Cout tiles to balance work

```diff
diff --git a/far3d_amd/csrc/conv_ws.hip b/far3d_amd/csrc/conv_ws.hip
--- a/far3d_amd/csrc/conv_ws.hip
+++ b/far3d_amd/csrc/conv_ws.hip
@@ -12,18 +12,18 @@
     case 401: return launch_conv3x3_ws<1, 8, 2, 1, 4, true, true>(P, st);
     case 402: return launch_conv3x3_ws<1, 8, 5, 1, 4, true, false>(P, st);
     case 403: return launch_conv3x3_ws<2, 4, 3, 1, 4, true, true>(P, st);
-    case 404: return launch_conv3x3_ws<2, 2, 1, 2, 2, true, true>(P, st);
-    case 405: return launch_conv3x3_ws<2, 4, 2, 1, 4, true, true>(P, st);
-    case 406: return launch_conv3x3_ws<2, 4, 1, 2, 4, true, true>(P, st);
+    case 404: return launch_conv3x3_ws<2, 2, 1, 2, 2, true, true, 3, false, 1, true>(P, st);
+    case 405: return launch_conv3x3_ws<2, 4, 2, 1, 4, true, true, 3, false, 1, true>(P, st);
+    case 406: return launch_conv3x3_ws<2, 4, 1, 2, 4, true, true, 3, false, 1, true>(P, st);
     case 407: return launch_conv3x3_ws<1, 4, 5, 1, 2, true, false>(P, st);
     case 408: return launch_conv3x3_ws<1, 4, 3, 1, 2, true, true>(P, st);
     case 409: return launch_conv3x3_ws<2, 4, 2, 2, 2, true, true>(P, st);
     case 410: return launch_conv3x3_ws<2, 4, 2, 2, 4, true, true, 4>(P, st);
     case 411: return launch_conv3x3_ws<2, 4, 2, 1, 4, true, true, 6>(P, st);
-    case 412: return launch_conv3x3_ws<2, 4, 1, 2, 4, true, true, 8>(P, st);
+    case 412: return launch_conv3x3_ws<2, 4, 1, 2, 4, true, true, 8, false, 1, true>(P, st);
     case 413: return launch_conv3x3_ws<1, 8, 2, 1, 4, true, true, 8>(P, st);
     case 414: return launch_conv3x3_ws<1, 4, 5, 1, 2, true, false, 5>(P, st);
-    case 415: return launch_conv3x3_ws<2, 2, 1, 2, 2, true, true, 6>(P, st);
+    case 415: return launch_conv3x3_ws<2, 2, 1, 2, 2, true, true, 6, false, 1, true>(P, st);
     case 416: return launch_conv3x3_ws<2, 4, 3, 1, 4, true, true, 4>(P, st);
     case 417: return launch_conv3x3_ws<2, 4, 2, 1, 4, true, true, 4>(P, st);
     case 418: return launch_conv3x3_ws<4, 2, 2, 2, 4, true, true, 3>(P, st);
@@ -31,24 +31,29 @@
     case 440: return launch_conv3x3_ws<2, 4, 2, 2, 4, true, true, 3, true>(P, st);
     case 444: return launch_conv3x3_ws<2, 2, 1, 2, 2, true, true, 3, true>(P, st);
     case 445: return launch_conv3x3_ws<2, 4, 2, 1, 4, true, true, 6, true>(P, st);
-    case 450: return launch_conv3x3_ws<2, 4, 2, 1, 4, true, true, 6, false, 3>(P, st);
-    case 451: return launch_conv3x3_ws<2, 4, 1, 2, 4, true, true, 6, false, 3>(P, st);
-    case 452: return launch_conv3x3_ws<2, 4, 1, 2, 4, true, true, 9, false, 3>(P, st);
-    case 453: return launch_conv3x3_ws<1, 8, 2, 1, 4, true, true, 6, false, 3>(P, st);
+    case 450: return launch_conv3x3_ws<2, 4, 2, 1, 4, true, true, 6, false, 3, true>(P, st);
+    case 451: return launch_conv3x3_ws<2, 4, 1, 2, 4, true, true, 6, false, 3, true>(P, st);
+    case 452: return launch_conv3x3_ws<2, 4, 1, 2, 4, true, true, 9, false, 3, true>(P, st);
+    case 453: return launch_conv3x3_ws<1, 8, 2, 1, 4, true, true, 6, false, 3, true>(P, st);
     case 454: return launch_conv3x3_ws<1, 8, 2, 1, 4, true, true, 9, false, 3>(P, st);
     case 455: return launch_conv3x3_ws<1, 7, 2, 1, 4, true, true, 9, false, 3>(P, st);
-    case 456: return launch_conv3x3_ws<2, 7, 1, 1, 2, true, true, 9, false, 3>(P, st);
-    case 457: return launch_conv3x3_ws<2, 2, 1, 2, 2, true, true, 6, false, 3>(P, st);
+    case 456: return launch_conv3x3_ws<2, 7, 1, 1, 2, true, true, 9, false, 3, true>(P, st);
+    case 457: return launch_conv3x3_ws<2, 2, 1, 2, 2, true, true, 6, false, 3, true>(P, st);
     case 458: return launch_conv3x3_ws<1, 4, 3, 1, 2, true, true, 6, false, 3>(P, st);
-    case 459: return launch_conv3x3_ws<2, 4, 1, 1, 4, true, true, 9, false, 3>(P, st);
+    case 459: return launch_conv3x3_ws<2, 4, 1, 1, 4, true, true, 9, false, 3, true>(P, st);
     case 420: return launch_conv3x3_ws<2, 4, 2, 2, 4, false, true>(P, st);
-    case 421: return launch_conv3x3_ws<1, 8, 2, 1, 4, false, true>(P, st);
+    case 421: return launch_conv3x3_ws<1, 8, 2, 1, 4, false, true, 3, false, 1, true>(P, st);
     case 422: return launch_conv3x3_ws<1, 8, 5, 1, 4, false, true>(P, st);
     case 423: return launch_conv3x3_ws<2, 4, 3, 1, 4, false, true>(P, st);
     default: break;
   }
   far3d_set_error("far3d_conv2d_nhwc: unknown wave-specialised tile %d", tile);
   return FAR3D_ERR_ARG;
+}
+
+extern "C" int far3d_ws_deal(int n_full, int n_light, int grid, int wg, int k) {
+  if (n_full < 0 || n_light < 0 || grid < 1 || wg < 0 || wg >= grid) return -1;
+  return ws_deal_item(n_full, n_light, grid, wg, k);
 }
 
 int far3d_gemm_ws_launch(const IgemmParams& P, int tile, hipStream_t st) {
@@ -79,9 +84,9 @@
   switch (tile) {
     case 500: return launch_conv3x3_ws_grouped<2, 4, 2, 2, 4, true, true>(P, G, st);
     case 505: return launch_conv3x3_ws_grouped<2, 4, 2, 1, 4, true, true>(P, G, st);
-    case 552: return launch_conv3x3_ws_grouped<2, 4, 1, 2, 4, true, true, 9, false, 3>(P, G, st);
-    case 556: return launch_conv3x3_ws_grouped<2, 7, 1, 1, 2, true, true, 9, false, 3>(P, G, st);
-    case 559: return launch_conv3x3_ws_grouped<2, 4, 1, 1, 4, true, true, 9, false, 3>(P, G, st);
+    case 552: return launch_conv3x3_ws_grouped<2, 4, 1, 2, 4, true, true, 9, false, 3, true>(P, G, st);
+    case 556: return launch_conv3x3_ws_grouped<2, 7, 1, 1, 2, true, true, 9, false, 3, true>(P, G, st);
+    case 559: return launch_conv3x3_ws_grouped<2, 4, 1, 1, 4, true, true, 9, false, 3, true>(P, G, st);
     default: break;
   }
   far3d_set_error("far3d_conv2d_nhwc_grouped: unknown grouped tile %d", tile);
diff --git a/far3d_amd/csrc/conv_ws.hpp b/far3d_amd/csrc/conv_ws.hpp
--- a/far3d_amd/csrc/conv_ws.hpp
+++ b/far3d_amd/csrc/conv_ws.hpp
@@ -40,7 +40,40 @@
 struct WsGroup { WsProblem p[FAR3D_WS_GROUP_MAX]; int n; };
 struct WsSingle {};
 
-template <int WGM, int WGN, int WM, int WN, int NP, bool PAIR, bool DBUF, int NSW = 3, bool FLAGS = false, int GRP = 1, class GT = WsSingle>
+#define FAR3D_WS_DEAL_FULL 2
+#define FAR3D_WS_DEAL_LIGHT 1
+struct WsDeal {
+  int F, G, b;
+  int nf, n1, n2;
+  int p, Nn, L1;
+};
+__host__ __device__ inline WsDeal ws_deal_prepare(int F, int L, int G, int b) {
+  WsDeal d;
+  d.F = F; d.G = G; d.b = b;
+  const int rem = F % G;
+  d.Nn = G - rem;
+  const int lvl = (FAR3D_WS_DEAL_FULL / FAR3D_WS_DEAL_LIGHT) * d.Nn;
+  d.L1 = rem ? (L < lvl ? L : lvl) : 0;
+  const int L2 = L - d.L1;
+  d.nf = F > b ? (F - b + G - 1) / G : 0;
+  d.p = b - rem;
+  d.n1 = (rem && d.p >= 0 && d.L1 > d.p) ? (d.L1 - d.p + d.Nn - 1) / d.Nn : 0;
+  d.n2 = L2 > b ? (L2 - b + G - 1) / G : 0;
+  return d;
+}
+__host__ __device__ inline int ws_deal_count(const WsDeal& d) { return d.nf + d.n1 + d.n2; }
+__host__ __device__ inline int ws_deal_at(const WsDeal& d, int k) {
+  if (k < 0) return -1;
+  if (k < d.nf) return d.b + k * d.G;
+  k -= d.nf;
+  if (k < d.n1) return d.F + d.p + k * d.Nn;
+  k -= d.n1;
+  return k < d.n2 ? d.F + d.L1 + d.b + k * d.G : -1;
+}
+__host__ __device__ inline int ws_deal_item(int F, int L, int G, int b, int k) { return ws_deal_at(ws_deal_prepare(F, L, G, b), k); }
+
+template <int WGM, int WGN, int WM, int WN, int NP, bool PAIR, bool DBUF, int NSW = 3, bool FLAGS = false, int GRP = 1, class GT = WsSingle,
+          bool DEFER = false>
 __global__ __launch_bounds__(64 * (WGM * WGN + NP)) void conv3x3_ws_kernel(IgemmParams P, int tiles_x, int tiles_y, int n_mt, int n_items, int ablate,
                                                                           GT GP) {
 #if defined(__HIP_DEVICE_COMPILE__)
@@ -70,7 +103,33 @@
   const int t = threadIdx.x, lane = t & 63, wv = __builtin_amdgcn_readfirstlane(t >> 6);
   const int nchunks = P.cin_pad / 32;
   const int spt = 9 * nchunks;
-  const int my_items = (n_items - (int)blockIdx.x + (int)gridDim.x - 1) / (int)gridDim.x;
+  static_assert(!DEFER || (!FLAGS && WM * WN * 16 <= 32), "the deferred epilogue: barrier hand-over, at most 32 accumulators per lane");
+  constexpr bool SKIP = WM * WN <= 2;
+  [[maybe_unused]] int deal_f = n_items, deal_l = 0;
+  if constexpr (!GROUPED && SKIP) {
+    if (P.Cout % BM) { deal_l = n_items / n_mt; deal_f = n_items - deal_l; }
+#ifdef FAR3D_PROFILING
+    if (ablate & 32) { deal_l = 0; deal_f = n_items; }
+#endif
+  }
+#ifdef FAR3D_PROFILING
+  const bool defer_on = DEFER && !(ablate & 16);
+#else
+  constexpr bool defer_on = DEFER;
+#endif
+  const WsDeal deal = ws_deal_prepare(deal_f, deal_l, (int)gridDim.x, (int)blockIdx.x);
+  const int my_items = GROUPED ? (n_items - (int)blockIdx.x + (int)gridDim.x - 1) / (int)gridDim.x : ws_deal_count(deal);
+  auto item_of = [&](int k, int& mt, int& pt) __attribute__((always_inline)) {
+    if constexpr (GROUPED) {
+      return (int)blockIdx.x + k * (int)gridDim.x;
+    } else {
+      const int o = ws_deal_at(deal, k);
+      if (deal_l == 0) { mt = o % n_mt; pt = o / n_mt; }
+      else if (o >= deal_f) { mt = n_mt - 1; pt = o - deal_f; }
+      else { const int nfm = n_mt - 1; mt = o % nfm; pt = o / nfm; }
+      return o;
+    }
+  };
   const int total_steps = my_items * spt, total_chunks = my_items * nchunks;
   const int Ktot = 9 * P.cin_pad * PLD;
   auto locate = [&](int item, int& q, int& li, int& txs, int& tys, int& nmt) __attribute__((always_inline)) {
@@ -111,10 +170,11 @@
     const bf16_t* w_base = nullptr;
     long w_bytes = 0;
     auto decode = [&](int k, int& n, int& y0, int& x0, int& m0, int& q) __attribute__((always_inline)) {
-      const int item = (int)blockIdx.x + k * (int)gridDim.x;
+      int mt = 0, pt = 0;
+      const int item = item_of(k, mt, pt);
       int li, txs, tys, nmt;
       locate(item, q, li, txs, tys, nmt);
-      const int mt = li % nmt, pt = li / nmt;
+      if constexpr (GROUPED) { mt = li % nmt; pt = li / nmt; }
       const int tx = pt % txs, r = pt / txs;
       const int ty = r % tys;
       n = __builtin_amdgcn_readfirstlane(r / tys); y0 = __builtin_amdgcn_readfirstlane(ty * TH);
@@ -127,7 +187,8 @@
       int Cout = P.Cout;
       if constexpr (GROUPED) { w = GP.p[q].w; Cout = GP.p[q].Cout; }
       w_base = reinterpret_cast<const bf16_t*>(w) + (long)m0 * Ktot;
-      w_bytes = w_tile_bytes(BM, m0, Cout, Ktot);
+      const int rows = Cout - m0;
+      w_bytes = (long)(rows < BM ? (rows > 0 ? rows : 0) : BM) * Ktot * 2;
     };
     auto set_p_tile = [&](int k) __attribute__((always_inline)) {
       int n, y0, x0, m0, q;
@@ -259,64 +320,150 @@
     }
   f32x16_t acc[WM][WN];
   u32x4_t fa[2][PLD][WM], fb[2][PLD][WN];
-
-  auto load_a = [&](int set, int soff, int kk) __attribute__((always_inline)) {
-#ifdef FAR3D_PROFILING
-    if (ablate & 4) return;
-#endif
-    const int x32 = kk * 32;
-#pragma unroll
-    for (int pl = 0; pl < PLD; ++pl)
-#pragma unroll
-      for (int i = 0; i < WM; ++i) fa[set][pl][i] = *reinterpret_cast<const u32x4_t*>(smem + pl * WST + ((aaddr[i] ^ x32) + soff));
+  int nv = WM;
+
+
+  auto epi_bias = [&](int i, int qp, int m0, int prob, float4 (&b4)[2]) __attribute__((always_inline)) {
+    const float* bias = P.bias;
+    int Cout = P.Cout;
+    if constexpr (GROUPED) { bias = GP.p[prob].bias; Cout = GP.p[prob].Cout; }
+    const int cb = m0 + (wm * WM + i) * 32;
+#pragma unroll
+    for (int u = 0; u < 2; ++u) {
+      b4[u] = make_float4(0.f, 0.f, 0.f, 0.f);
+      if (bias && cb < Cout) b4[u] = *reinterpret_cast<const float4*>(bias + cb + 8 * (2 * qp + u) + 4 * hi);
+    }
   };
-  auto load_b = [&](int set, int tap, int kk) __attribute__((always_inline)) {
-#ifdef FAR3D_PROFILING
-    if (ablate & 4) return;
-#endif
-    const int ky = tap / 3, kx = tap - 3 * ky, x32 = kk * 32;
-#pragma unroll
-    for (int pl = 0; pl < PLD; ++pl)
-#pragma unroll
-      for (int j = 0; j < WN; ++j) fb[set][pl][j] = *reinterpret_cast<const u32x4_t*>(smem + pl * PATCH_B + (baddr[j + ky][kx] ^ x32));
+  auto epi_slice = [&](auto biased_tag, const f32x16_t (&A)[WM][WN], int i, int j, int qp, int n, int y0, int x0, int m0, int prob,
+                       const float4 (*b4)[2] = nullptr) __attribute__((always_inline)) {
+    constexpr bool BIASED = decltype(biased_tag)::value;
+    const int px = x0 + l31;
+    void* y = P.y;
+    long yis = P.y_img_stride;
+    int Ho = P.Ho, Wo = P.Wo, ldy = P.ldy, Cout = P.Cout, act = P.act;
+    [[maybe_unused]] float* y2 = nullptr;
+    [[maybe_unused]] const float *y2s = nullptr, *y2h = nullptr;
+    [[maybe_unused]] long y2is = 0;
+    [[maybe_unused]] int ldy2 = 0;
+    if constexpr (GROUPED) {
+      const WsProblem& pq = GP.p[prob];
+      y = pq.y; yis = pq.y_img_stride; Ho = pq.H; Wo = pq.W; ldy = pq.ldy; Cout = pq.Cout; act = pq.act;
+      y2 = pq.y2; y2s = pq.y2_scale; y2h = pq.y2_shift; y2is = pq.y2_img_stride; ldy2 = pq.ldy2;
+    }
+    unsigned char* yb = reinterpret_cast<unsigned char*>(y);
+    const int py = y0 + wn * WN + j;
+    const bool ok = py < Ho && px < Wo;
+    const long pix_b = ((long)n * yis + ((long)py * Wo + px) * ldy) * 2;
+    const int cb = m0 + (wm * WM + i) * 32;
+    if (cb >= Cout) return;
+    uint2 h[2], l[2];
+#pragma unroll
+    for (int u = 0; u < 2; ++u) {
+      const int q = 2 * qp + u;
+      float v[4];
+#pragma unroll
+      for (int e = 0; e < 4; ++e) v[e] = A[i][j][4 * q + e];
+      if constexpr (!BIASED) { const float4 bq = (*b4)[u]; v[0] += bq.x; v[1] += bq.y; v[2] += bq.z; v[3] += bq.w; }
+      if (act == ACT_RELU) {
+#pragma unroll
+        for (int e = 0; e < 4; ++e) v[e] = fmaxf(v[e], 0.f);
+      } else if (act == ACT_SWISH) {
+        if constexpr (PAIR) {
+#pragma unroll
+          for (int e = 0; e < 4; ++e) v[e] = v[e] * (1.f / (1.f + expf(-v[e])));
+        } else {
+#pragma unroll
+          for (int e = 0; e < 4; ++e) v[e] = v[e] * __frcp_rn(1.f + __expf(-v[e]));
+        }
+      }
+      if constexpr (GROUPED) {
+        if (y2 && ok) {
+          const int m = cb + 8 * q + 4 * hi;
+          const long so = (long)n * Cout + m;
+          float w4[4];
+#pragma unroll
+          for (int e = 0; e < 4; ++e) w4[e] = y2s[so + e] * v[e] + y2h[so + e];
+          *reinterpret_cast<float4*>(y2 + n * y2is + ((long)py * Wo + px) * ldy2 + m) = make_float4(w4[0], w4[1], w4[2], w4[3]);
+        }
+      }
+      if constexpr (PAIR) split4f(v[0], v[1], v[2], v[3], h[u], l[u]);
+      else { h[u] = make_uint2(pack_bf16x2(v[0], v[1]), pack_bf16x2(v[2], v[3])); l[u] = make_uint2(0u, 0u); }
+    }
+    u32x4_t oh, ol;
+    {
+      const auto sx = __builtin_amdgcn_permlane32_swap(h[0].x, h[1].x, false, false);
+      const auto sy = __builtin_amdgcn_permlane32_swap(h[0].y, h[1].y, false, false);
+      oh = u32x4_t{sx[0], sy[0], sx[1], sy[1]};
+    }
+    const int qoff = (2 * qp + hi) * 16;
+    if constexpr (PAIR) {
+      const auto sx = __builtin_amdgcn_permlane32_swap(l[0].x, l[1].x, false, false);
+      const auto sy = __builtin_amdgcn_permlane32_swap(l[0].y, l[1].y, false, false);
+      ol = u32x4_t{sx[0], sy[0], sx[1], sy[1]};
+      if (ok) {
+        unsigned char* d = yb + pix_b + (long)(cb >> 5) * 128 + qoff;
+        *reinterpret_cast<u32x4_t*>(d) = oh;
+        *reinterpret_cast<u32x4_t*>(d + 64) = ol;
+      }
+    } else {
+      if (ok) *reinterpret_cast<u32x4_t*>(yb + pix_b + (long)cb * 2 + qoff) = oh;
+    }
   };
-  auto load_set = [&](int set, int soff, int tap, int kk) __attribute__((always_inline)) { load_a(set, soff, kk); load_b(set, tap, kk); };
-  auto mma_term = [&](int set, int term) __attribute__((always_inline)) {
-    const int pa = (PAIR && term == 0) ? 1 : 0, pb = (PAIR && term == 1) ? 1 : 0;
-#pragma unroll
-    for (int i = 0; i < WM; ++i)
-#pragma unroll
-      for (int j = 0; j < WN; ++j) mma<bf16_t>(acc[i][j], fa[set][pa][i], fb[set][pb][j]);
-  };
-  auto mma_set = [&](int set) __attribute__((always_inline)) {
-    if constexpr (PAIR) { mma_term(set, 0); mma_term(set, 1); }
-    mma_term(set, 2);
-  };
+  constexpr int NSL = WM * WN * 2, NHG = 9 / GRP, SPG = (NSL + NHG - 1) / NHG;
+  [[maybe_unused]] f32x16_t pacc[DEFER ? WM : 1][DEFER ? WN : 1];
+  [[maybe_unused]] int pd_n = 0, pd_y0 = 0, pd_x0 = 0, pd_m0 = 0, pd_prob = 0;
 
   int G = 0;
   int soff = 0;
   [[maybe_unused]] int Sg = 0;
   [[maybe_unused]] u32x4_t pfl = {0u, 0u, 0u, 0u};
 #ifdef FAR3D_PROFILING
-  unsigned long long pf_ta = 0, pf_tb = 0, pf_wait = 0, pf_body = 0, pf_epi = 0;
+  unsigned long long pf_ta = 0, pf_tb = 0, pf_wait = 0, pf_body = 0, pf_epi = 0, pf_dg = 0;
   const bool pf_on = P.prof != nullptr && wv == 0;
 #endif
-  for (int k = 0; k < my_items; ++k) {
-    const int item = (int)blockIdx.x + k * (int)gridDim.x;
-    int prob, li, txs, tys, nmt;
-    locate(item, prob, li, txs, tys, nmt);
-    const int mt = li % nmt, pt = li / nmt;
-    const int tx = pt % txs, rr = pt / txs;
-    const int ty = rr % tys, n = rr / tys;
-    const int x0 = tx * 32, y0 = ty * TH, m0 = mt * BM;
-#pragma unroll
-    for (int i = 0; i < WM; ++i)
-#pragma unroll
-      for (int j = 0; j < WN; ++j)
-#pragma unroll
-        for (int r = 0; r < 16; ++r) acc[i][j][r] = 0.f;
-
-    for (int c = 0; c < nchunks; ++c, ++G) {
+  auto run_chunks = [&](auto nvc_tag, int k) __attribute__((always_inline)) {
+    constexpr int NVC = decltype(nvc_tag)::value;
+    auto slice_on = [&](int i) __attribute__((always_inline)) { return i < NVC; };
+
+    auto load_a = [&](int set, int soff, int kk) __attribute__((always_inline)) {
+#ifdef FAR3D_PROFILING
+      if (ablate & 4) return;
+#endif
+      const int x32 = kk * 32;
+#pragma unroll
+      for (int pl = 0; pl < PLD; ++pl)
+#pragma unroll
+        for (int i = 0; i < WM; ++i)
+          if (slice_on(i)) fa[set][pl][i] = *reinterpret_cast<const u32x4_t*>(smem + pl * WST + ((aaddr[i] ^ x32) + soff));
+    };
+    auto load_b = [&](int set, int tap, int kk) __attribute__((always_inline)) {
+#ifdef FAR3D_PROFILING
+      if (ablate & 4) return;
+#endif
+      if (!slice_on(0)) return;
+      const int ky = tap / 3, kx = tap - 3 * ky, x32 = kk * 32;
+#pragma unroll
+      for (int pl = 0; pl < PLD; ++pl)
+#pragma unroll
+        for (int j = 0; j < WN; ++j) fb[set][pl][j] = *reinterpret_cast<const u32x4_t*>(smem + pl * PATCH_B + (baddr[j + ky][kx] ^ x32));
+    };
+    auto load_set = [&](int set, int soff, int tap, int kk) __attribute__((always_inline)) { load_a(set, soff, kk); load_b(set, tap, kk); };
+    auto mma_term = [&](int set, int term) __attribute__((always_inline)) {
+      const int pa = (PAIR && term == 0) ? 1 : 0, pb = (PAIR && term == 1) ? 1 : 0;
+#pragma unroll
+      for (int i = 0; i < WM; ++i)
+        if (slice_on(i)) {
+#pragma unroll
+          for (int j = 0; j < WN; ++j) mma<bf16_t>(acc[i][j], fa[set][pa][i], fb[set][pb][j]);
+        }
+    };
+    auto mma_set = [&](int set) __attribute__((always_inline)) {
+      if constexpr (PAIR) { mma_term(set, 0); mma_term(set, 1); }
+      mma_term(set, 2);
+    };
+
+    auto chunk = [&](auto first_tag) __attribute__((always_inline)) {
+      constexpr bool FIRST = decltype(first_tag)::value;
 #pragma unroll
       for (int tap = 0; tap < 9; ++tap) {
         const int stage = soff;
@@ -325,7 +472,7 @@
 #ifdef FAR3D_PROFILING
         if (pf_on) {
           const unsigned long long now = __builtin_amdgcn_s_memtime();
-          if (pf_tb) { pf_wait += pf_tb - pf_ta; pf_body += now - pf_tb; }
+          if (pf_tb) { pf_wait += pf_tb - pf_ta; pf_body += now - pf_tb - pf_dg; pf_dg = 0; }
           pf_ta = now;
         }
 #endif
@@ -354,14 +501,14 @@
         __builtin_amdgcn_sched_barrier(0);
 #ifdef FAR3D_PROFILING
         if (pf_on) pf_tb = __builtin_amdgcn_s_memtime();
-        if (tap == 0 && c == 0 && k == 0 && P.prof && t == 0) P.prof[(long)blockIdx.x * 16 + 2] = (unsigned long long)__builtin_amdgcn_s_memtime();
+        if (tap == 0 && FIRST && k == 0 && P.prof && t == 0) P.prof[(long)blockIdx.x * 16 + 2] = (unsigned long long)__builtin_amdgcn_s_memtime();
 #endif
         }
         if (ablate & 2) { soff = soff == (NSW - 1) * WSTAGE ? 0 : soff + WSTAGE; continue; }
         if constexpr (DBUF) {
           load_set(0, stage, tap, 0);
           __builtin_amdgcn_sched_barrier(0);
-          if (tap > 0 || c > 0) mma_set(1);
+          if (tap > 0 || !FIRST) mma_set(1);
           __builtin_amdgcn_sched_barrier(0);
           load_a(1, stage, 1);
           if constexpr (FLAGS) pfl = *reinterpret_cast<volatile u32x4_t*>(smem + FLAGB);
@@ -392,107 +539,101 @@
           __builtin_amdgcn_sched_barrier(0);
           soff = soff == (NSW - 1) * WSTAGE ? 0 : soff + WSTAGE;
         }
+        if constexpr (DEFER) {
+          if (tap % GRP == GRP - 1 && k > 0 && FIRST && defer_on) {
+#ifdef FAR3D_PROFILING
+            unsigned long long pf_d0 = 0;
+            if (pf_on) pf_d0 = __builtin_amdgcn_s_memtime();
+#endif
+#pragma unroll
+            for (int u = 0; u < SPG; ++u) {
+              const int sl = (tap / GRP) * SPG + u;
+              if (sl < NSL) epi_slice(std::true_type{}, pacc, (sl >> 1) % WM, (sl >> 1) / WM, sl & 1, pd_n, pd_y0, pd_x0, pd_m0, pd_prob);
+            }
+            __builtin_amdgcn_sched_barrier(0);
+#ifdef FAR3D_PROFILING
+            if (pf_on) { const unsigned long long dd = __builtin_amdgcn_s_memtime() - pf_d0; pf_epi += dd; pf_dg += dd; }
+#endif
+          }
+        }
       }
       const int d = (G & 1) ? -PBUF : PBUF;
 #pragma unroll
       for (int r = 0; r < RB; ++r)
 #pragma unroll
         for (int kx = 0; kx < 3; ++kx) baddr[r][kx] += d;
-    }
+    };
+    chunk(std::true_type{});
+    ++G;
+#pragma unroll 1
+    for (int c = 1; c < nchunks; ++c, ++G) chunk(std::false_type{});
     if constexpr (DBUF) mma_set(1);
+  };
+  for (int k = 0; k < my_items; ++k) {
+    int mt = 0, pt = 0;
+    const int item = item_of(k, mt, pt);
+    int prob, li, txs, tys, nmt;
+    locate(item, prob, li, txs, tys, nmt);
+    if constexpr (GROUPED) { mt = li % nmt; pt = li / nmt; }
+    const int tx = pt % txs, rr = pt / txs;
+    const int ty = rr % tys, n = rr / tys;
+    const int x0 = tx * 32, y0 = ty * TH, m0 = mt * BM;
+    {
+      int Cout = P.Cout;
+      if constexpr (GROUPED) Cout = GP.p[prob].Cout;
+      const int left = (Cout - m0) / 32 - wm * WM;
+      nv = __builtin_amdgcn_readfirstlane(left < 0 ? 0 : (left > WM ? WM : left));
+    }
+#pragma unroll
+    for (int i = 0; i < WM; ++i)
+#pragma unroll
+      for (int j = 0; j < WN; ++j)
+#pragma unroll
+        for (int r = 0; r < 16; ++r) acc[i][j][r] = 0.f;
+
+    if constexpr (SKIP) {
+      if (nv == WM) run_chunks(std::integral_constant<int, WM>{}, k);
+      else if (WM == 2 && nv == 1) run_chunks(std::integral_constant<int, 1>{}, k);
+      else run_chunks(std::integral_constant<int, 0>{}, k);
+    } else {
+      run_chunks(std::integral_constant<int, WM>{}, k);
+    }
     __builtin_amdgcn_sched_barrier(0);
 #ifdef FAR3D_PROFILING
     unsigned long long pf_e0 = 0;
     if (pf_on) {
       pf_e0 = __builtin_amdgcn_s_memtime();
-      if (pf_tb) { pf_wait += pf_tb - pf_ta; pf_body += pf_e0 - pf_tb; pf_tb = 0; }
-    }
-#endif
-
-    {
-      const int px = x0 + l31;
-      void* y = P.y;
-      const float* bias = P.bias;
-      long yis = P.y_img_stride;
-      int Ho = P.Ho, Wo = P.Wo, ldy = P.ldy, Cout = P.Cout, act = P.act;
-      [[maybe_unused]] float* y2 = nullptr;
-      [[maybe_unused]] const float *y2s = nullptr, *y2h = nullptr;
-      [[maybe_unused]] long y2is = 0;
-      [[maybe_unused]] int ldy2 = 0;
-      if constexpr (GROUPED) {
-        const WsProblem& pq = GP.p[prob];
-        y = pq.y; bias = pq.bias; yis = pq.y_img_stride; Ho = pq.H; Wo = pq.W; ldy = pq.ldy; Cout = pq.Cout; act = pq.act;
-        y2 = pq.y2; y2s = pq.y2_scale; y2h = pq.y2_shift; y2is = pq.y2_img_stride; ldy2 = pq.ldy2;
-      }
-      unsigned char* yb = reinterpret_cast<unsigned char*>(y);
-#pragma unroll
-      for (int j = 0; j < WN; ++j) {
-        const int py = y0 + wn * WN + j;
-        const bool ok = py < Ho && px < Wo;
-        const long pix_b = ((long)n * yis + ((long)py * Wo + px) * ldy) * 2;
-#pragma unroll
-        for (int i = 0; i < WM; ++i) {
-          const int cb = m0 + (wm * WM + i) * 32;
-          if (cb >= Cout) continue;
+      if (pf_tb) { pf_wait += pf_tb - pf_ta; pf_body += pf_e0 - pf_tb - pf_dg; pf_dg = 0; pf_tb = 0; }
+    }
+#endif
+
+    if (defer_on && k + 1 < my_items) {
+#pragma unroll
+      for (int i = 0; i < WM; ++i) {
+        float4 b4[2][2];
+        epi_bias(i, 0, m0, prob, b4[0]);
+        epi_bias(i, 1, m0, prob, b4[1]);
+#pragma unroll
+        for (int j = 0; j < WN; ++j)
+#pragma unroll
+          for (int q = 0; q < 4; ++q) {
+            const float4 bq = b4[q >> 1][q & 1];
+            pacc[i][j][4 * q + 0] = acc[i][j][4 * q + 0] + bq.x; pacc[i][j][4 * q + 1] = acc[i][j][4 * q + 1] + bq.y;
+            pacc[i][j][4 * q + 2] = acc[i][j][4 * q + 2] + bq.z; pacc[i][j][4 * q + 3] = acc[i][j][4 * q + 3] + bq.w;
+          }
+      }
+      pd_n = n; pd_y0 = y0; pd_x0 = x0; pd_m0 = m0; pd_prob = prob;
+    } else {
+#pragma unroll
+      for (int j = 0; j < WN; ++j)
+#pragma unroll
+        for (int i = 0; i < WM; ++i)
 #pragma unroll
           for (int qp = 0; qp < 2; ++qp) {
-            uint2 h[2], l[2];
-#pragma unroll
-            for (int u = 0; u < 2; ++u) {
-              const int q = 2 * qp + u;
-              float4 b4 = make_float4(0.f, 0.f, 0.f, 0.f);
-              if (bias) b4 = *reinterpret_cast<const float4*>(bias + cb + 8 * q + 4 * hi);
-              float v[4];
-#pragma unroll
-              for (int e = 0; e < 4; ++e) v[e] = acc[i][j][4 * q + e];
-              v[0] += b4.x; v[1] += b4.y; v[2] += b4.z; v[3] += b4.w;
-              if (act == ACT_RELU) {
-#pragma unroll
-                for (int e = 0; e < 4; ++e) v[e] = fmaxf(v[e], 0.f);
-              } else if (act == ACT_SWISH) {
-                if constexpr (PAIR) {
-#pragma unroll
-                  for (int e = 0; e < 4; ++e) v[e] = v[e] * (1.f / (1.f + expf(-v[e])));
-                } else {
-#pragma unroll
-                  for (int e = 0; e < 4; ++e) v[e] = v[e] * __frcp_rn(1.f + __expf(-v[e]));
-                }
-              }
-              if constexpr (GROUPED) {
-                if (y2 && ok) {
-                  const int m = cb + 8 * q + 4 * hi;
-                  const long so = (long)n * Cout + m;
-                  float w4[4];
-#pragma unroll
-                  for (int e = 0; e < 4; ++e) w4[e] = y2s[so + e] * v[e] + y2h[so + e];
-                  *reinterpret_cast<float4*>(y2 + n * y2is + ((long)py * Wo + px) * ldy2 + m) = make_float4(w4[0], w4[1], w4[2], w4[3]);
-                }
-              }
-              if constexpr (PAIR) split4f(v[0], v[1], v[2], v[3], h[u], l[u]);
-              else { h[u] = make_uint2(pack_bf16x2(v[0], v[1]), pack_bf16x2(v[2], v[3])); l[u] = make_uint2(0u, 0u); }
-            }
-            u32x4_t oh, ol;
-            {
-              const auto sx = __builtin_amdgcn_permlane32_swap(h[0].x, h[1].x, false, false);
-              const auto sy = __builtin_amdgcn_permlane32_swap(h[0].y, h[1].y, false, false);
-              oh = u32x4_t{sx[0], sy[0], sx[1], sy[1]};
-            }
-            const int qoff = (2 * qp + hi) * 16;
-            if constexpr (PAIR) {
-              const auto sx = __builtin_amdgcn_permlane32_swap(l[0].x, l[1].x, false, false);
-              const auto sy = __builtin_amdgcn_permlane32_swap(l[0].y, l[1].y, false, false);
-              ol = u32x4_t{sx[0], sy[0], sx[1], sy[1]};
-              if (ok) {
-                unsigned char* d = yb + pix_b + (long)(cb >> 5) * 128 + qoff;
-                *reinterpret_cast<u32x4_t*>(d) = oh;
-                *reinterpret_cast<u32x4_t*>(d + 64) = ol;
-              }
-            } else {
-              if (ok) *reinterpret_cast<u32x4_t*>(yb + pix_b + (long)cb * 2 + qoff) = oh;
-            }
+            float4 b4[2];
+            epi_bias(i, qp, m0, prob, b4);
+            epi_slice(std::false_type{}, acc, i, j, qp, n, y0, x0, m0, prob, &b4);
           }
-        }
-      }
     }
 #ifdef FAR3D_PROFILING
     if (pf_on) pf_epi += __builtin_amdgcn_s_memtime() - pf_e0;
@@ -926,7 +1067,7 @@
   return 0;
 }
 
-template <int WGM, int WGN, int WM, int WN, int NP, bool PAIR, bool DBUF, int NSW = 3, bool FLAGS = false, int GRP = 1>
+template <int WGM, int WGN, int WM, int WN, int NP, bool PAIR, bool DBUF, int NSW = 3, bool FLAGS = false, int GRP = 1, bool DEFER = false>
 static int launch_conv3x3_ws(const IgemmParams& P, hipStream_t st) {
   constexpr int BM = 32 * WGM * WM, TH = WGN * WN, PLD = PAIR ? 2 : 1;
   constexpr int PG = (34 * (TH + 2) + 15) / 16;
@@ -946,13 +1087,13 @@
   const int grid = n_items < cus * wg_per_cu ? n_items : cus * wg_per_cu;
   static std::atomic<unsigned long long> lds_ok{0};
   if constexpr (lds > 65536)
-    if (const int rc = far3d_allow_lds(reinterpret_cast<const void*>(&conv3x3_ws_kernel<WGM, WGN, WM, WN, NP, PAIR, DBUF, NSW, FLAGS, GRP>), (int)lds, lds_ok, "far3d_conv2d_nhwc")) return rc;
-  hipLaunchKernelGGL((conv3x3_ws_kernel<WGM, WGN, WM, WN, NP, PAIR, DBUF, NSW, FLAGS, GRP>), dim3((unsigned)grid), dim3(64 * (WGM * WGN + NP)), lds, st, P, tiles_x, tiles_y, n_mt,
+    if (const int rc = far3d_allow_lds(reinterpret_cast<const void*>(&conv3x3_ws_kernel<WGM, WGN, WM, WN, NP, PAIR, DBUF, NSW, FLAGS, GRP, WsSingle, DEFER>), (int)lds, lds_ok, "far3d_conv2d_nhwc")) return rc;
+  hipLaunchKernelGGL((conv3x3_ws_kernel<WGM, WGN, WM, WN, NP, PAIR, DBUF, NSW, FLAGS, GRP, WsSingle, DEFER>), dim3((unsigned)grid), dim3(64 * (WGM * WGN + NP)), lds, st, P, tiles_x, tiles_y, n_mt,
                      n_items, FAR3D_WS_ABLATE_ARG, WsSingle{});
   return 0;
 }
 
-template <int WGM, int WGN, int WM, int WN, int NP, bool PAIR, bool DBUF, int NSW = 3, bool FLAGS = false, int GRP = 1>
+template <int WGM, int WGN, int WM, int WN, int NP, bool PAIR, bool DBUF, int NSW = 3, bool FLAGS = false, int GRP = 1, bool DEFER = false>
 static int launch_conv3x3_ws_grouped(const IgemmParams& P, const WsGroup& G0, hipStream_t st) {
   constexpr int BM = 32 * WGM * WM, TH = WGN * WN, PLD = PAIR ? 2 : 1;
   constexpr int PG = (34 * (TH + 2) + 15) / 16;
@@ -985,9 +1126,9 @@
   const int grid = n_items < cus * wg_per_cu ? (int)n_items : cus * wg_per_cu;
   static std::atomic<unsigned long long> lds_ok{0};
   if constexpr (lds > 65536)
-    if (const int rc = far3d_allow_lds(reinterpret_cast<const void*>(&conv3x3_ws_kernel<WGM, WGN, WM, WN, NP, PAIR, DBUF, NSW, FLAGS, GRP, WsGroup>), (int)lds, lds_ok,
+    if (const int rc = far3d_allow_lds(reinterpret_cast<const void*>(&conv3x3_ws_kernel<WGM, WGN, WM, WN, NP, PAIR, DBUF, NSW, FLAGS, GRP, WsGroup, DEFER>), (int)lds, lds_ok,
                                        "far3d_conv2d_nhwc_grouped")) return rc;
-  hipLaunchKernelGGL((conv3x3_ws_kernel<WGM, WGN, WM, WN, NP, PAIR, DBUF, NSW, FLAGS, GRP, WsGroup>), dim3((unsigned)grid), dim3(64 * (WGM * WGN + NP)), lds, st, P,
+  hipLaunchKernelGGL((conv3x3_ws_kernel<WGM, WGN, WM, WN, NP, PAIR, DBUF, NSW, FLAGS, GRP, WsGroup, DEFER>), dim3((unsigned)grid), dim3(64 * (WGM * WGN + NP)), lds, st, P,
                      G.p[0].tiles_x, G.p[0].tiles_y, G.p[0].n_mt, (int)n_items, FAR3D_WS_ABLATE_ARG, G);
   return 0;
 }
diff --git a/far3d_amd/lib.py b/far3d_amd/lib.py
--- a/far3d_amd/lib.py
+++ b/far3d_amd/lib.py
@@ -24,6 +24,7 @@
                           [c_long] + [c_int] * 5 + [_p, c_int, c_int, c_long, c_int, c_int] +
                           [_p, c_int, c_int, c_long, _p, _p, _p, c_int, _p]),
     "far3d_conv2d_nhwc_grouped": (c_int, [_p, c_int, c_int, _p]),
+    "far3d_ws_deal": (c_int, [c_int] * 5),
     "far3d_attention_forward": (c_int, [_p, _p, _p, c_int, _p, c_int] + [c_int] * 8 + [c_float, _p, c_int, c_int, _p]),
     "far3d_attention_f32_variant": (c_int, [c_int]),
     "far3d_layernorm": (c_int, [_p, _p, _p, _p, c_int, c_int, c_int, c_int, c_float, c_int, _p, c_int, _p, c_int, c_int, _p, c_int, c_int, _p]),
diff --git a/include/far3d_hip.h b/include/far3d_hip.h
--- a/include/far3d_hip.h
+++ b/include/far3d_hip.h
@@ -63,6 +63,8 @@
 
 int far3d_conv2d_nhwc_grouped(const far3d_conv_problem* probs, int n, int tile, void* stream);
 
+int far3d_ws_deal(int n_full, int n_light, int grid, int wg, int k);
+
 int far3d_attention_forward(const void* q, const void* k, const void* v, int dtype, void* out, int out_dt, int Aq, int Nk,
                             int heads, int head_dim, int ldq, int ldk, int ldv, int ldo, float scale,
                             const int32_t* hole_count, int hole_start, int hole_end, void* stream);
```

Measured after the change: 74.14 samples/s, median of 6. 2.6% higher.
